# aluo-x/3D_SLN

Measured on AMD Instinct MI355X. Metric: scene-graph VAE steps/sec + 256² diff-render fps, 1/2/4/8 MI355X, higher is better.
Workload: dtype f32; 1 GPU; BASELINE configs[1]: batch=64 scene graphs x (32 objects, 64 triples) per GPU, Sg2ScVAE train step at train.py defaults (embedding_dim=64, 5+5 GraphTripleConv, BatchNorm); O=2048, T=4096, hipgraph=True, distinct_batches_cycled=4, eps=N(0,1) drawn on the device inside the step, parallelism=dp1

## Files before the change

### 3d_sln_amd/_lib.py

```python
from __future__ import annotations

import ctypes as C
import os

HERE = os.path.dirname(os.path.abspath(__file__))
LIB_PATH = os.path.join(HERE, "libsln_hip.so")

SLN_E = {-1: "SLN_E_BADARG", -2: "SLN_E_UNSUPPORTED", -3: "SLN_E_STATE", -4: "SLN_E_NOGPU", -5: "SLN_E_NOMEM", -6: "SLN_E_CAPTURE"}

c_f32p = C.c_void_p
c_i64p = C.c_void_p


class SlnError(RuntimeError):
    pass


class SlnVaeConfig(C.Structure):
    _fields_ = [(n, C.c_int) for n in (
        "embedding_dim", "gconv_num_layers", "recurrent", "batch_norm", "decoder_cat", "use_ae",
        "box_dim", "n_angle", "num_objs", "num_preds", "num_attrs", "no_attr")]


class SlnVaeUnit(C.Structure):
# ... 115 lines not shown
class SlnDbgEmbed(C.Structure):
    _fields_ = [(n, C.c_void_p) for n in ("objs", "attrs", "angles", "boxes", "obj_emb", "attr_emb", "angle_emb", "wb", "bb", "mu", "logvar", "eps",
                                          "z_in", "z", "x0", "dx0", "d_obj_emb", "d_attr_emb", "d_angle_emb", "d_wb", "d_bb", "dz", "idx", "src",
                                          "dst", "src2", "dst2", "st_objs", "st_attrs", "st_angles", "st_boxes", "attrs32", "deg", "err",
                                          "zero_ptr")] + [("zero_bytes", C.c_int64)] + \
               [(n, C.c_int) for n in ("kind", "O", "n_obj", "n_attr", "n_box", "n_angle", "box_dim", "n_z", "use_ae", "z_in_x0", "rows_obj",
                                       "rows_attr", "rows_angle", "ld", "col0", "n", "table_rows", "T", "n2", "pad_")]


class SlnDbgOpt(C.Structure):
    _fields_ = [(n, C.c_void_p) for n in ("params", "grads", "m", "v", "total_loss")] + [("pro", C.POINTER(SlnDbgEmbed))] + \
               [("n", C.c_int64), ("step", C.c_int64), ("seed", C.c_uint64), ("offset", C.c_uint64)] + \
               [(n, C.c_float) for n in ("lr", "beta1", "beta2", "eps")] + [("kind", C.c_int), ("calls", C.c_int)] + \
               [("out_step", C.c_int64), ("out_offset", C.c_uint64), ("out_bc1", C.c_float), ("out_bc2", C.c_float), ("out_skip", C.c_int),
                ("pad_", C.c_int)]


class SlnViewPlace(C.Structure):
    _fields_ = [(n, C.c_void_p) for n in ("bank_v", "bank_f", "voff", "foff", "voff_host", "foff_host", "A", "tr", "row_model", "row_label",
                                          "shell_v", "shell_f", "shell_f_host", "shell_label", "K", "Rm", "t")] + \
               [(n, C.c_int32) for n in ("M", "Vtot", "Ftot", "Fm", "Vs", "Fs", "R", "V", "N", "reserved")] + \
               [("orig_size", C.c_float), ("near", C.c_float)]


class SlnReproject(C.Structure):
    _fields_ = [(n, C.c_void_p) for n in ("depth_src", "k_src", "pose", "K_tgt")] + \
               [(n, C.c_int32) for n in ("B", "Hs", "Ws", "reserved")] + \
               [(n, C.c_float) for n in ("orig_size", "near", "gap", "reserved_f")]


class SlnDraw3D(C.Structure):
    _fields_ = [(n, C.c_void_p) for n in ("faces_xyz", "face_index", "depth", "face_label", "chosen", "K", "light_cam", "albedo")] + \
               [(n, C.c_int32) for n in ("R", "V", "F", "S", "k", "shadows")] + \
               [(n, C.c_float) for n in ("ambient", "intensity", "min_dist", "bias")] + [("background", C.c_float * 3)]


SIGNATURES = {
    "sln_version": (C.c_int, []),
    "sln_build_arch": (C.c_char_p, []),
    "sln_device_ok": (C.c_int, []),
    "sln_vae_num_units": (C.c_int, [C.POINTER(SlnVaeConfig)]),
    "sln_vae_create": (C.c_int, [C.POINTER(SlnVaeConfig), C.POINTER(C.c_void_p)]),
    "sln_vae_destroy": (None, [C.c_void_p]),
    "sln_vae_workspace_bytes": (C.c_int64, [C.c_void_p, C.c_int, C.c_int]),
    "sln_vae_bind": (C.c_int, [C.c_void_p, C.POINTER(SlnVaeTensors), C.c_void_p, C.c_int64, C.c_int, C.c_int]),
    "sln_vae_set_batch": (C.c_int, [C.c_void_p, C.POINTER(SlnVaeBatch), C.c_void_p]),
    "sln_vae_check_batch": (C.c_int, [C.c_void_p, C.c_void_p]),
    "sln_vae_encoder": (C.c_int, [C.c_void_p, c_f32p, c_f32p, C.c_int, C.c_void_p]),
    "sln_vae_decoder": (C.c_int, [C.c_void_p, c_f32p, c_f32p, c_f32p, C.c_int, C.c_void_p]),
    "sln_vae_forward": (C.c_int, [C.c_void_p, c_f32p, c_f32p, c_f32p, c_f32p, c_f32p, c_f32p, C.c_int, C.c_void_p]),
    "sln_vae_loss": (C.c_int, [C.c_void_p, c_f32p, c_f32p, c_f32p, c_f32p, C.c_float, c_f32p, C.c_int, C.c_void_p]),
    "sln_vae_decoder_backward": (C.c_int, [C.c_void_p, c_f32p, c_f32p, c_f32p, C.c_void_p]),
    "sln_vae_encoder_backward": (C.c_int, [C.c_void_p, c_f32p, c_f32p, C.c_void_p]),
    "sln_vae_backward": (C.c_int, [C.c_void_p, C.c_void_p]),
    "sln_vae_params_changed": (C.c_int, [C.c_void_p]),
    "sln_vae_zero_grad": (C.c_int, [C.c_void_p, C.c_void_p]),
    "sln_vae_adam_step": (C.c_int, [C.c_void_p, C.c_float, C.c_void_p]),
    "sln_vae_adam_reset": (C.c_int, [C.c_void_p, C.c_int64, C.c_void_p]),
    "sln_vae_adam_get_step": (C.c_int, [C.c_void_p, C.POINTER(C.c_int64), C.c_void_p]),
    "sln_vae_set_grad_guard": (C.c_int, [C.c_void_p, c_f32p]),
    "sln_vae_seed": (C.c_int, [C.c_void_p, C.c_uint64, C.c_uint64, C.c_void_p]),
    "sln_vae_last_eps": (C.c_int, [C.c_void_p, c_f32p, C.c_void_p]),
    "sln_vae_randn": (C.c_int, [C.c_void_p, c_f32p, C.c_int64, C.c_void_p]),
    "sln_layout_heatmap": (C.c_int, [c_f32p, C.c_int64, C.c_int, C.c_int, C.c_int, C.c_int, c_f32p, C.c_void_p]),
    "sln_vae_set_training": (C.c_int, [C.c_void_p, C.c_int]),
    "sln_vae_set_gemm_precision": (C.c_int, [C.c_void_p, C.c_int]),
    "sln_vae_train_step": (C.c_int, [C.c_void_p, c_f32p, C.c_float, C.c_float, c_f32p, C.c_int, C.c_int, C.c_void_p]),
    "sln_vae_group_create": (C.c_int, [C.POINTER(C.c_void_p), C.c_int, C.POINTER(SlnVaeGroupIO), C.POINTER(C.c_void_p)]),
    "sln_vae_group_decoder": (C.c_int, [C.c_void_p, C.c_void_p]),
    "sln_vae_group_decoder_backward": (C.c_int, [C.c_void_p, C.c_void_p]),
    "sln_vae_group_launches": (C.c_int, [C.c_void_p, C.POINTER(C.c_int), C.POINTER(C.c_int), C.POINTER(C.c_int)]),
    "sln_vae_group_transposes": (C.c_int64, [C.c_void_p]),
    "sln_vae_group_fused_params": (C.c_int, [C.c_void_p, C.POINTER(C.c_void_p), C.POINTER(C.c_int64), C.c_int]),
    "sln_vae_group_destroy": (None, [C.c_void_p]),
    "sln_debug_side_stream": (C.c_int, [C.c_void_p, C.POINTER(C.c_int), C.POINTER(C.c_int)]),
    "sln_side_stream_prepare": (C.c_int, [C.c_void_p]),
    "sln_side_stream_forget": (C.c_int, [C.c_void_p]),
    "sln_prof_enable": (C.c_int, [C.c_int]),
    "sln_set_deterministic": (C.c_int, [C.c_int]),
    "sln_get_deterministic": (C.c_int, []),
    "sln_set_store_policy": (C.c_int, [C.c_int]),
    "sln_get_store_policy": (C.c_int, []),
    "sln_parse_store_policy_env": (C.c_int, [C.c_char_p, C.c_int]),
    "sln_debug_tn_plan": (C.c_int, [C.c_void_p, C.c_void_p, C.c_void_p, C.c_int, C.c_void_p, C.c_void_p, C.c_int]),
    "sln_debug_tn_plan_mixed": (C.c_int, [C.c_void_p, C.c_void_p, C.c_void_p, C.c_void_p, C.c_int, C.c_void_p, C.c_void_p, C.c_int]),
    "sln_prof_read": (C.c_int, [C.c_void_p, C.c_void_p, C.c_void_p, C.c_int]),
    "sln_vae_tap": (C.c_int64, [C.c_void_p, C.c_int, C.c_int, c_f32p, C.c_void_p]),
    "sln_gconv_workspace_bytes": (C.c_int64, [C.c_int, C.c_int, C.c_int, C.c_int, C.c_int, C.c_int]),
    "sln_gconv_forward": (C.c_int, [C.c_int, C.c_int, C.c_int, C.c_int, C.c_int, C.c_int, C.POINTER(SlnVaeUnit), c_f32p, c_f32p,
                                    C.c_void_p, C.c_int, C.c_int, C.c_int, C.c_void_p, C.c_int64, c_f32p, c_f32p, C.c_void_p]),
    "sln_gconv_net_create": (C.c_int, [C.c_int, C.c_int, C.c_int, C.c_int, C.c_int, C.c_int, C.POINTER(C.c_void_p)]),
    "sln_gconv_net_set_edges": (C.c_int, [C.c_void_p, C.c_void_p, C.c_int, C.c_int, C.c_void_p]),
    "sln_gconv_net_forward": (C.c_int, [C.c_void_p, c_f32p, c_f32p, c_f32p, c_f32p, C.c_int, C.c_void_p]),
    "sln_gconv_net_backward": (C.c_int, [C.c_void_p, c_f32p, c_f32p, c_f32p, c_f32p, C.c_void_p]),
    "sln_linear_forward": (C.c_int, [c_f32p, C.c_int, C.c_int, c_f32p, c_f32p, c_f32p, C.c_int, C.c_void_p,
                                     C.c_int, C.c_void_p]),
    "sln_linear_wgrad": (C.c_int, [c_f32p, c_f32p, C.c_int, C.c_int, C.c_int, c_f32p, c_f32p, C.c_void_p]),
    "sln_debug_gemm_nt": (C.c_int, [C.POINTER(SlnDbgGemmNT), C.c_int, C.POINTER(C.c_int), C.c_void_p]),
    "sln_debug_gemm_tn": (C.c_int, [C.POINTER(SlnDbgGemmTN), C.c_int, C.c_int, C.c_void_p]),
    "sln_debug_gemm_tn_mixed": (C.c_int, [C.POINTER(SlnDbgGemmTN), C.c_int, C.c_void_p]),
    "sln_debug_gemm_nt_route": (C.c_int, [C.POINTER(SlnDbgGemmNT), C.POINTER(SlnDbgNTRoute)]),
    "sln_debug_gemm_nt_half": (C.c_int, [C.POINTER(SlnDbgGemmNT), C.c_int, C.c_void_p]),
    "sln_debug_gemm_nt_half_takes": (C.c_int, [C.POINTER(SlnDbgGemmNT)]),
    "sln_debug_gemm_sizes": (C.c_int, [C.POINTER(C.c_int), C.c_int]),
    "sln_debug_vae_csr": (C.c_int, [c_i64p, C.c_int, C.c_int, C.c_int, C.POINTER(SlnDbgCsr), C.c_void_p, C.c_void_p]),
    "sln_debug_vae_edge": (C.c_int, [C.POINTER(SlnDbgEdge), C.c_int, C.c_int, C.POINTER(C.c_int), C.c_void_p]),
    "sln_debug_vae_loss": (C.c_int, [C.POINTER(SlnDbgLoss), C.c_void_p]),
    "sln_debug_vae_tables": (C.c_int, [C.c_int, C.c_void_p, C.c_int, C.c_int, C.c_float, C.c_int, C.c_int, C.c_int, C.c_void_p]),
    "sln_debug_vae_embed": (C.c_int, [C.POINTER(SlnDbgEmbed), C.c_int, C.c_int, C.POINTER(C.c_int), C.c_void_p]),
    "sln_debug_vae_opt": (C.c_int, [C.POINTER(SlnDbgOpt), C.c_void_p]),
    "sln_debug_vae_sizes": (C.c_int, [C.POINTER(C.c_int), C.c_int]),
    "sln_debug_vae_leaf_launches": (C.c_int64, [C.c_void_p]),
    "sln_debug_vae_half_launches": (C.c_int64, [C.c_void_p]),
    "sln_debug_vae_tail_launches": (C.c_int64, [C.c_void_p]),
    "sln_debug_vae_graph_captures": (C.c_int64, [C.c_void_p]),
    "sln_project_faces": (C.c_int, [c_f32p, C.c_void_p, c_f32p, c_f32p, c_f32p, C.c_int, C.c_int, C.c_int, C.c_float, C.c_float, c_f32p, C.c_void_p]),
    "sln_project_faces_backward": (C.c_int, [c_f32p, C.c_void_p, c_f32p, c_f32p, c_f32p, C.c_int, C.c_int, C.c_int, C.c_float, C.c_float, c_f32p,
                                             c_f32p, C.c_void_p]),
    "sln_raster_workspace_bytes": (C.c_int64, [C.c_int, C.c_int]),
    "sln_raster_forward": (C.c_int, [c_f32p, C.c_int, C.c_int, C.c_int, C.c_float, C.c_float, C.c_void_p, C.c_void_p,
                                     c_f32p, c_f32p, C.c_void_p]),
    "sln_raster_forward_dual": (C.c_int, [c_f32p, C.c_int, C.c_int, C.c_int, C.c_float, C.c_float, C.c_float, C.c_void_p,
                                          C.c_void_p, c_f32p, c_f32p, C.c_void_p, c_f32p, c_f32p, C.c_void_p]),
    "sln_raster_texture_sample": (C.c_int, [c_f32p, c_f32p, C.c_void_p, c_f32p, c_f32p, C.c_int, C.c_int, C.c_int, C.c_int,
                                            C.c_float, c_f32p, C.c_void_p]),
    "sln_raster_backward_depth": (C.c_int, [c_f32p, C.c_void_p, c_f32p, c_f32p, c_f32p, C.c_int, C.c_int, C.c_int, c_f32p,
                                            C.c_void_p]),
    "sln_raster_backward_rgb": (C.c_int, [c_f32p, C.c_void_p, c_f32p, c_f32p, C.c_int, C.c_int, C.c_int, C.c_int, C.c_float,
                                          c_f32p, C.c_void_p]),
    "sln_raster_texture_sample_chw": (C.c_int, [c_f32p, c_f32p, C.c_void_p, c_f32p, c_f32p, C.c_int, C.c_int, C.c_int, C.c_int, C.c_int,
                                                C.c_float, C.c_float, c_f32p, C.c_void_p]),
    "sln_raster_backward_rgb_multi": (C.c_int, [c_f32p, C.c_void_p, C.c_void_p, C.c_void_p, C.c_int, C.c_int, C.c_int, C.c_int, C.c_float,
                                                C.c_void_p, c_f32p, C.c_void_p]),
    "sln_scene_workspace_bytes": (C.c_int64, [C.c_int, C.c_int, C.c_int]),
    "sln_scene_forward": (C.c_int, [c_f32p, C.c_void_p, C.c_int, C.c_int, C.c_int, C.c_int, C.c_void_p, C.c_void_p,
                                    C.c_float, C.c_float, C.c_float, C.c_float, C.c_void_p, c_f32p, C.c_void_p]),
    "sln_scene_forward_live": (C.c_int, [c_f32p, C.c_void_p, C.c_int, C.c_int, C.c_int, C.c_int, C.c_void_p, C.c_void_p,
                                         C.c_float, C.c_float, C.c_float, C.c_float, C.c_void_p, c_f32p, C.c_void_p, C.c_void_p, C.c_void_p]),
    "sln_spade_prepare": (C.c_int, [C.c_void_p]),
    "sln_spade_release": (C.c_int, [C.c_void_p, C.c_int]),
    "sln_spade_conv": (C.c_int, [c_f32p, C.c_int, C.c_int, C.c_int, C.c_int, c_f32p, c_f32p, C.c_int, C.c_int, C.c_int, C.c_int,
                                 C.c_float, c_f32p, C.c_void_p]),
    "sln_spade_modulate": (C.c_int, [c_f32p, C.c_int, C.c_int, C.c_int, C.c_int, c_f32p, c_f32p, C.c_int, C.c_int, c_f32p, c_f32p,
                                     C.c_int, C.c_float, c_f32p, C.c_void_p]),
    "sln_layernorm_stats": (C.c_int, [c_f32p, C.c_int, C.c_int64, C.c_float, C.c_void_p, c_f32p, C.c_void_p]),
    "sln_spade_apply": (C.c_int, [c_f32p, c_f32p, C.c_int, C.c_int, C.c_int, C.c_int, C.c_int, c_f32p, C.c_int, C.c_float, c_f32p, C.c_void_p]),
    "sln_spade_apply_up": (C.c_int, [c_f32p, C.c_int, c_f32p, C.c_int, C.c_int, C.c_int, C.c_int, C.c_int, c_f32p, C.c_int, C.c_float, c_f32p,
                                     C.c_void_p]),
    "sln_resize": (C.c_int, [c_f32p, C.c_int, C.c_int, C.c_int, C.c_int, C.c_int, C.c_int, c_f32p, C.c_void_p]),
    "sln_spade_depth_concat": (C.c_int, [c_f32p, C.c_int, C.c_int, C.c_int, C.c_int, c_f32p, c_f32p, C.c_int, c_f32p, C.c_int, C.c_void_p]),
    "sln_se_scale_add": (C.c_int, [c_f32p, c_f32p, C.c_int, C.c_int, C.c_int64, c_f32p, c_f32p, c_f32p, c_f32p, C.c_void_p]),
    "sln_spade_conv_sums": (C.c_int, [c_f32p, C.c_int, C.c_int, C.c_int, C.c_int, c_f32p, c_f32p, C.c_int, C.c_int, C.c_int, C.c_int,
                                      C.c_float, c_f32p, C.c_void_p, C.c_void_p, C.c_void_p]),
    "sln_spade_modulate_up": (C.c_int, [c_f32p, C.c_int, C.c_int, C.c_int, C.c_int, c_f32p, c_f32p, C.c_int, C.c_int, c_f32p, C.c_int,
                                        c_f32p, C.c_int, C.c_float, c_f32p, C.c_void_p]),
    "sln_layernorm_finalize": (C.c_int, [C.c_void_p, C.c_int, C.c_int64, C.c_int, C.c_float, c_f32p, C.c_void_p]),
    "sln_spade_conv_f16": (C.c_int, [c_f32p, C.c_int, C.c_int, C.c_int, C.c_int, C.c_void_p, C.c_void_p, c_f32p, C.c_int, C.c_int, C.c_int,
                                     C.c_int, C.c_float, c_f32p, C.c_void_p]),
    "sln_spade_conv_sums_f16": (C.c_int, [c_f32p, C.c_int, C.c_int, C.c_int, C.c_int, C.c_void_p, C.c_void_p, c_f32p, C.c_int, C.c_int,
                                          C.c_int, C.c_int, C.c_float, c_f32p, C.c_void_p, C.c_void_p, C.c_void_p]),
    "sln_spade_modulate_f16": (C.c_int, [c_f32p, C.c_int, C.c_int, C.c_int, C.c_int, C.c_void_p, C.c_void_p, c_f32p, C.c_int, C.c_int,
                                         c_f32p, c_f32p, C.c_int, C.c_float, c_f32p, C.c_void_p]),
    "sln_spade_modulate_up_f16": (C.c_int, [c_f32p, C.c_int, C.c_int, C.c_int, C.c_int, C.c_void_p, C.c_void_p, c_f32p, C.c_int, C.c_int,
                                            c_f32p, C.c_int, c_f32p, C.c_int, C.c_float, c_f32p, C.c_void_p]),
    "sln_block_tail": (C.c_int, [c_f32p, C.c_int, c_f32p, C.c_int, C.c_int, C.c_int, C.c_int, C.c_void_p, c_f32p, c_f32p, c_f32p,
                                 C.c_int, c_f32p, C.c_void_p, C.c_int, C.c_float, c_f32p, C.c_void_p]),
# ... 122 lines not shown
```

### 3d_sln_amd/csrc/gemm_bodies.h

```cpp
#pragma once
#include "sln_common.h"
#include "sln_gemm.h"
#include "sln_prof.h"

#include <cstdlib>
#include <cstring>
#include <type_traits>
namespace {


#ifndef SLN_TRACE
#define SLN_TRACE(i)
#endif
#ifndef SLN_TRACEH
#define SLN_TRACEH(i)
#endif

#ifndef SLN_NT_SCHED
#define SLN_NT_SCHED 1
#endif
#ifndef SLN_TN_SCHED
#define SLN_TN_SCHED 1
#endif
#ifndef SLN_TN_ABL
// ... 1237 lines not shown
        if (n == 0) pieceG(rt, buf, 0, stage_next);
        if (n == 1) pieceG2(rt, 0, stage_next);
        if (n == 2) pieceG(rt, buf, 1, stage_next);
        if (n == 3) { pieceG2(rt, 1, stage_next); rd(buf, 2, S0{}); }
      });
      mma4(S1{}, [&](int n) __attribute__((always_inline)) {
        if (n == 0) pieceX(rt, buf, 0, stage_next);
        if (n == 1) pieceX(rt, buf, 1, stage_next);
        if (n == 2) pieceI(rt, 0, stage_next);
        if (n == 3) { pieceI(rt, 1, stage_next); rd(buf, 3, S1{}); }
      });
      mma4(S0{}, [&](int) __attribute__((always_inline)) {});
      __syncthreads();
      rd(buf ^ 1, 0, S0{});
      SLN_SB;
      mma4(S1{}, [&](int) __attribute__((always_inline)) {});
    };
#undef SLN_SB
    for (int rt = 0; rt < ntiles; rt += 2) { sbody(rt, S1{}); sbody(rt + 1, S0{}); }
  }
#else
  for (int rt = 0; rt < ntiles; rt += 2) { body(rt, S1{}); body(rt + 1, S0{}); }
#endif

  __syncthreads();
  float* red = As;
  {
    float* dst = red + (wave * 16) * 64 + lane;
    if (wr == 0) {
#pragma unroll
      for (int r = 0; r < 16; ++r) dst[r * 64] = tn_acc_read(acc[1][r]);
    } else {
#pragma unroll
      for (int r = 0; r < 16; ++r) dst[r * 64] = tn_acc_read(acc[0][r]);
    }
  }
  __syncthreads();
  {
    const float* src = red + ((wave ^ 2) * 16) * 64 + lane;
    const float sc = a.sgd_step != nullptr ? -a.sgd_step[0] : 1.f;
    const int k = k0 + 32 * wc + lrow;
    float* dcol = a.dW + min(k, a.Kin - 1);
    const bool kv = k < a.Kin;
    if (wr == 0) {
#pragma unroll
      for (int r = 0; r < 16; ++r) {
        const float v = (tn_acc_read(acc[0][r]) + src[r * 64]) * sc;
        const int n = n0 + 2 * ((r & 3) + 8 * (r >> 2) + 4 * lk);
        if (kv && n < a.Nout) sln_gatomic_add(dcol + (size_t)n * a.lddw, v);
      }
    } else {
#pragma unroll
      for (int r = 0; r < 16; ++r) {
        const float v = (src[r * 64] + tn_acc_read(acc[1][r])) * sc;
        const int n = n0 + 2 * ((r & 3) + 8 * (r >> 2) + 4 * lk) + 1;
        if (kv && n < a.Nout) sln_gatomic_add(dcol + (size_t)n * a.lddw, v);
      }
    }
  }

  if (a.db != nullptr && (bx % tiles_k) == 0) {
#pragma unroll
    for (int off = TPRA; off < 64; off <<= 1) {
      dbacc.x += __shfl_xor(dbacc.x, off, 64); dbacc.y += __shfl_xor(dbacc.y, off, 64);
      dbacc.z += __shfl_xor(dbacc.z, off, 64); dbacc.w += __shfl_xor(dbacc.w, off, 64);
    }
    __syncthreads();
    float4* dbs = reinterpret_cast<float4*>(red);
    if (lane < TPRA) dbs[wave * TPRA + lane] = dbacc;
    __syncthreads();
    if (tid < TPRA) {
      const float4 p0 = dbs[tid], p1 = dbs[TPRA + tid], p2 = dbs[2 * TPRA + tid], p3 = dbs[3 * TPRA + tid];
      const int n = n0 + 4 * tid;
      const float sb = a.sgd_step != nullptr ? -a.sgd_step[0] : 1.f;
      if (n + 0 < a.Nout) sln_gatomic_add(a.db + n + 0, (((p0.x + p1.x) + p2.x) + p3.x) * sb);
      if (n + 1 < a.Nout) sln_gatomic_add(a.db + n + 1, (((p0.y + p1.y) + p2.y) + p3.y) * sb);
      if (n + 2 < a.Nout) sln_gatomic_add(a.db + n + 2, (((p0.z + p1.z) + p2.z) + p3.z) * sb);
      if (n + 3 < a.Nout) sln_gatomic_add(a.db + n + 3, (((p0.w + p1.w) + p2.w) + p3.w) * sb);
    }
  }
}


template <bool G_X2>
__device__ __forceinline__ void gemm_tn_mixed_item(const GemmTNArgs* __restrict__ probs, const TnMultiItem it, char* smem) {
  if (it.prob < 0) return;
  if (it.xg) gemm_tn_body<64, 64, 2, 2, G_X2, true>(probs[it.prob], it.tile, it.chunk, smem);
  else gemm_tn_body<64, 64, 2, 2, G_X2, false>(probs[it.prob], it.tile, it.chunk, smem);
}

inline bool tn_gathers(const GemmTNArgs& a) {
  bool g = false;
  for (int s = 0; s < a.X.nseg; ++s) g |= a.X.seg[s].which != 0;
  return g;
}

inline bool tn_supported(const GemmTNArgs& a) {
  for (int s = 0; s < a.G.nseg; ++s) if (a.G.seg[s].which != 0) return false;
  return true;
}

inline size_t nt_smem_bytes(int K, int BM, int BN, int WM) {
  const int kpad = (K + 31) & ~31;
  return (size_t)sln_crows(kpad + 4) * 16 + (size_t)2 * (BM + BN) * (BK + 4) * 4 + (size_t)BN * 16 + (size_t)WM * BN * 16;
}

inline size_t tn_smem_bytes(int BM, int BN) { return (size_t)(BM + BN) * 16 + (size_t)2 * BK * (BM + TN_PAD + BN + TN_PAD) * 4; }

inline int nt_heuristic_tile(const GemmNTArgs& a) {
  static const int forced = std::getenv("SLN_NT_TILE") ? std::atoi(std::getenv("SLN_NT_TILE")) : -1;
  (void)a;
  return forced >= 0 ? forced : 0;
}

inline bool nt_big_shape(const GemmNTArgs& a) {
  return (long)sln_cdiv(a.M, 128) * sln_cdiv(a.N, 64) >= 384;
}

inline bool nt_unaligned(const GemmNTArgs& a) {
  for (int s = 0; s + 1 < a.A.nseg; ++s) if (a.A.seg[s].len % BK) return true;
  return false;
}

inline int nt_amode(const GemmNTArgs& a) {
  bool x2 = false;
  for (int s = 0; s < a.A.nseg; ++s) x2 |= a.A.seg[s].x2 != nullptr;
  bool ident = !x2;
  for (int s = 0; s < a.A.nseg; ++s) ident = ident && a.A.seg[s].coef == SLN_COEF_IDENT;
  return x2 ? 1 : (ident ? 2 : 0);
}

inline bool tn_prepare(GemmTNArgs& a) {
  bool x2 = false;
  for (int s = 0; s < a.G.nseg; ++s) x2 |= a.G.seg[s].x2 != nullptr;
  if (a.rows_per_block <= 0) {
    static const int target = std::getenv("SLN_TN_TARGET") ? std::atoi(std::getenv("SLN_TN_TARGET")) : 768;
    static const int minrows = std::getenv("SLN_TN_MINROWS") ? std::atoi(std::getenv("SLN_TN_MINROWS")) : 256;
    const int tiles = sln_cdiv(a.Nout, 64) * sln_cdiv(a.Kin, 64);
    int chunks = sln_cdiv(target, tiles);
    int rpb = sln_cdiv(sln_cdiv(a.R, chunks), BK) * BK;
    a.rows_per_block = rpb < minrows ? minrows : rpb;
  }
  return x2;
}

}
```

### 3d_sln_amd/csrc/gemm_f32.hip

```cpp
#include <cstdio>
#include <cstdlib>
#include <algorithm>
#include <vector>
#include "gemm_bodies.h"
#include "vae_multi.h"
namespace {
constexpr bool nt_coef_helpers(int amode, int epi) { return amode != 2 || epi == EPI_MASK; }
template <int BM, int BN, int AMODE, int EPI>
constexpr bool nt_helpers() { return BM == 64 && BN == 64 && nt_coef_helpers(AMODE, EPI); }
template <int BM, int BN, int WM, int WN, int AMODE, int EPI, int MULTI, int ST = 0>
__global__ __launch_bounds__((nt_helpers<BM, BN, AMODE, EPI>() ? 512 : 256)) void gemm_nt_kernel(const GemmNTArgs a) {
  extern __shared__ __attribute__((aligned(16))) char smem[];
  gemm_nt_body<BM, BN, WM, WN, AMODE, EPI, MULTI, nt_helpers<BM, BN, AMODE, EPI>(), ST>(a, blockIdx.x, ((a.M + BM - 1) / BM) * ((a.N + BN - 1) / BN), smem);
}

template <int AMODE, int EPI>
constexpr bool nt_helpers2() { return nt_coef_helpers(AMODE, EPI); }
template <int J, int AMODE, int EPI, int ST = 0>
__global__ __launch_bounds__((nt_helpers2<AMODE, EPI>() ? 512 : 256)) void gemm_nt16_kernel(const GemmNTArgs a) {
  extern __shared__ __attribute__((aligned(16))) char smem[];
  gemm_nt_body16<J, AMODE, EPI, nt_helpers2<AMODE, EPI>(), ST>(a, blockIdx.x, ((a.M + 63) / 64) * ((a.N + 32 * J - 1) / (32 * J)), smem);
}

template <int AMODE, int EPI, int NSEG = 1, int ST = 0>
// ... 51 lines not shown
  else hipLaunchKernelGGL((gemm_nt16_kernel<J, AMODE, EPI>), dim3(grid), dim3(nt_helpers2<AMODE, EPI>() ? 512 : 256), smem, st, a);
  SLN_CHECK_LAUNCH();
  return 0;
}

template <int BM, int BN, int WM, int WN, int AMODE, int EPI>
int launch_nt(const GemmNTArgs& a, const NtRoute& rt, hipStream_t st) {
  const size_t smem = nt_smem_bytes(a.K, BM, BN, WM);
  const int grid = sln_cdiv(a.M, BM) * sln_cdiv(a.N, BN);
  if (grid <= 0) return 0;
  if (smem > 48 * 1024) { int r = sln_gemm_init(); if (r) return r; }
  constexpr int NTHR = nt_helpers<BM, BN, AMODE, EPI>() ? 512 : 256;
  if (rt.threads != NTHR) return -3;
#define SLN_NT_GO(ST_)                                                                                                                   \
  if (rt.multi == 2) {                                                                                                                   \
    if constexpr (BM == 64 && BN == 64) hipLaunchKernelGGL((gemm_nt_kernel<64, 64, WM, WN, AMODE, EPI, 2, ST_>), dim3(grid), dim3(NTHR), smem, st, a); \
    else return -2;                                          \
  }                                                                                                                                      \
  else if (rt.multi == 1) hipLaunchKernelGGL((gemm_nt_kernel<BM, BN, WM, WN, AMODE, EPI, 1, ST_>), dim3(grid), dim3(NTHR), smem, st, a); \
  else hipLaunchKernelGGL((gemm_nt_kernel<BM, BN, WM, WN, AMODE, EPI, 0, ST_>), dim3(grid), dim3(NTHR), smem, st, a);
  if (nt_store_mode() == SLN_ST_WT) { SLN_NT_GO(SLN_ST_WT) } else { SLN_NT_GO(SLN_ST_PLAIN) }
#undef SLN_NT_GO
  SLN_CHECK_LAUNCH();
  return 0;
}

template <int AMODE, int EPI>
int launch_nt_route(const GemmNTArgs& a, const NtRoute& rt, hipStream_t st) {
  switch (rt.body) {
    case NT_BODY_SMALL: return launch_nt_small<AMODE, EPI>(a, rt, st);
    case NT_BODY_SMALL3: return launch_nt_small<AMODE, EPI, 3>(a, rt, st);
    case NT_BODY_16J3: return launch_nt16<3, AMODE, EPI>(a, rt, st);
    case NT_BODY_16J5: return launch_nt16<5, AMODE, EPI>(a, rt, st);
    case NT_BODY_128x64: return launch_nt<128, 64, 2, 2, AMODE, EPI>(a, rt, st);
    case NT_BODY_128: return launch_nt<128, 128, 2, 2, AMODE, EPI>(a, rt, st);
    case NT_BODY_64: return launch_nt<64, 64, 2, 2, AMODE, EPI>(a, rt, st);
    default: return -1;
  }
}

NtRoute nt_route(const GemmNTArgs& a, int epi, int tile) {
  static const bool no_small = std::getenv("SLN_NO_SMALL_NT") != nullptr;
  NtRoute r;
  r.amode = nt_amode(a); r.multi = 0;
  if (tile < 0 && !no_small && nt_wants_small(a)) r.body = NT_BODY_SMALL;
  else if (tile < 0 && !no_small && nt_wants_small3(a)) { r.body = NT_BODY_SMALL3; r.multi = 1; }
  else {
    const int J16 = tile < 0 ? nt16_pick(a) : 0;
    if (J16 == 3) r.body = NT_BODY_16J3;
    else if (J16 == 5) r.body = NT_BODY_16J5;
    else {
      if (tile < 0) tile = nt_heuristic_tile(a);
      const bool unaligned = a.A.nseg > 1 && nt_unaligned(a);
      if (unaligned) tile = 0;
      r.body = tile == 1 ? NT_BODY_128x64 : (tile == 2 ? NT_BODY_128 : NT_BODY_64);
      r.multi = a.A.nseg > 1 ? (unaligned ? 2 : 1) : 0;
    }
  }
  const bool big = r.body == NT_BODY_128x64 || r.body == NT_BODY_128;
  r.threads = !big && nt_coef_helpers(r.amode, epi) ? 512 : 256;
  return r;
}

template <int BM, int BN, int WM, int WN, bool G_X2, bool XG>
__global__ __launch_bounds__(256) void gemm_tn_kernel(const GemmTNArgs a) {
  extern __shared__ __attribute__((aligned(16))) char smem[];
  gemm_tn_body<BM, BN, WM, WN, G_X2, XG>(a, blockIdx.x, blockIdx.y, smem);
}

template <bool G_X2, bool XG>
__global__ __launch_bounds__(256) void gemm_tn_multi_kernel(const GemmTNArgs* __restrict__ probs, const TnMultiMeta* __restrict__ meta) {
  extern __shared__ __attribute__((aligned(16))) char smem[];
  const TnMultiItem it = meta->item[blockIdx.x];
  if (it.prob < 0) return;
  gemm_tn_body<64, 64, 2, 2, G_X2, XG>(probs[it.prob], it.tile, it.chunk, smem);
}

template <bool G_X2>
__global__ __launch_bounds__(256) void gemm_tn_mixed_kernel(const GemmTNArgs* __restrict__ probs, const TnMixedMeta* __restrict__ meta) {
  extern __shared__ __attribute__((aligned(16))) char smem[];
  gemm_tn_mixed_item<G_X2>(probs, meta->item[blockIdx.x], smem);
}

template <int BM, int BN, int WM, int WN, bool G_X2>
int launch_tn(const GemmTNArgs& a, hipStream_t st) {
  const size_t smem = tn_smem_bytes(BM, BN);
  const int gx = sln_cdiv(a.Nout, BM) * sln_cdiv(a.Kin, BN);
  const int gy = sln_cdiv(a.R, a.rows_per_block);
  if (gx <= 0 || gy <= 0) return 0;
  if (!tn_supported(a)) return -1;
  if (tn_gathers(a)) hipLaunchKernelGGL((gemm_tn_kernel<BM, BN, WM, WN, G_X2, true>), dim3(gx, gy), dim3(256), smem, st, a);
  else hipLaunchKernelGGL((gemm_tn_kernel<BM, BN, WM, WN, G_X2, false>), dim3(gx, gy), dim3(256), smem, st, a);
  SLN_CHECK_LAUNCH();
  return 0;
}

}

template <int BM, int BN, int WM, int WN, int ST>
static int init_nt_tile() {
  hipError_t e = hipSuccess;
#define SLN_SET(X2, EPI)                                                                                          \
  if (e == hipSuccess)                                                                                            \
    e = hipFuncSetAttribute(reinterpret_cast<const void*>(&gemm_nt_kernel<BM, BN, WM, WN, X2, EPI, 0, ST>),       \
                            hipFuncAttributeMaxDynamicSharedMemorySize, 160 * 1024);                              \
  if (e == hipSuccess)                                                                                            \
    e = hipFuncSetAttribute(reinterpret_cast<const void*>(&gemm_nt_kernel<BM, BN, WM, WN, X2, EPI, 1, ST>),       \
                            hipFuncAttributeMaxDynamicSharedMemorySize, 160 * 1024);                              \
  if (e == hipSuccess && BM == 64 && BN == 64)                                                                    \
    e = hipFuncSetAttribute(reinterpret_cast<const void*>(&gemm_nt_kernel<64, 64, WM, WN, X2, EPI, 2, ST>),       \
                            hipFuncAttributeMaxDynamicSharedMemorySize, 160 * 1024);
  SLN_SET(0, EPI_PLAIN) SLN_SET(0, EPI_STATS) SLN_SET(0, EPI_MASK)
  SLN_SET(1, EPI_PLAIN) SLN_SET(1, EPI_STATS) SLN_SET(1, EPI_MASK)
  SLN_SET(2, EPI_PLAIN) SLN_SET(2, EPI_STATS) SLN_SET(2, EPI_MASK)
#undef SLN_SET
  return (int)e;
}

int sln_gemm_group_init();
int sln_vae_tail_init();
int sln_gemm_init() {
  static bool done = false;
  if (done) return 0;
  int r = init_nt_tile<64, 64, 2, 2, SLN_ST_PLAIN>();
  if (!r) r = init_nt_tile<64, 64, 2, 2, SLN_ST_WT>();
#define SLN_SET_S(AM, EPI)                                                                                        \
  if (!r) r = (int)hipFuncSetAttribute(reinterpret_cast<const void*>(&gemm_nt_small_kernel<AM, EPI, 1>),         \
                                       hipFuncAttributeMaxDynamicSharedMemorySize, 160 * 1024);                  \
  if (!r) r = (int)hipFuncSetAttribute(reinterpret_cast<const void*>(&gemm_nt_small_kernel<AM, EPI, 3>),         \
                                       hipFuncAttributeMaxDynamicSharedMemorySize, 160 * 1024);                  \
  if (!r) r = (int)hipFuncSetAttribute(reinterpret_cast<const void*>(&gemm_nt_small_kernel<AM, EPI, 1, SLN_ST_WT>), \
                                       hipFuncAttributeMaxDynamicSharedMemorySize, 160 * 1024);                  \
  if (!r) r = (int)hipFuncSetAttribute(reinterpret_cast<const void*>(&gemm_nt_small_kernel<AM, EPI, 3, SLN_ST_WT>), \
                                       hipFuncAttributeMaxDynamicSharedMemorySize, 160 * 1024);
  SLN_SET_S(0, EPI_PLAIN) SLN_SET_S(0, EPI_STATS) SLN_SET_S(0, EPI_MASK) SLN_SET_S(1, EPI_PLAIN) SLN_SET_S(1, EPI_STATS)
  SLN_SET_S(1, EPI_MASK) SLN_SET_S(2, EPI_PLAIN) SLN_SET_S(2, EPI_STATS) SLN_SET_S(2, EPI_MASK)
#undef SLN_SET_S
#define SLN_SET_16(J, AM, EPI)                                                                                    \
  if (!r) r = (int)hipFuncSetAttribute(reinterpret_cast<const void*>(&gemm_nt16_kernel<J, AM, EPI>),             \
                                       hipFuncAttributeMaxDynamicSharedMemorySize, 160 * 1024);                  \
  if (!r) r = (int)hipFuncSetAttribute(reinterpret_cast<const void*>(&gemm_nt16_kernel<J, AM, EPI, SLN_ST_WT>),  \
                                       hipFuncAttributeMaxDynamicSharedMemorySize, 160 * 1024);
#define SLN_SET_16J(J)                                                                                            \
  SLN_SET_16(J, 0, EPI_PLAIN) SLN_SET_16(J, 0, EPI_STATS) SLN_SET_16(J, 0, EPI_MASK) SLN_SET_16(J, 1, EPI_PLAIN) SLN_SET_16(J, 1, EPI_STATS) \
  SLN_SET_16(J, 1, EPI_MASK) SLN_SET_16(J, 2, EPI_PLAIN) SLN_SET_16(J, 2, EPI_STATS) SLN_SET_16(J, 2, EPI_MASK)
  SLN_SET_16J(3) SLN_SET_16J(5)
#undef SLN_SET_16J
#undef SLN_SET_16
  if (!r) r = init_nt_tile<128, 64, 2, 2, SLN_ST_PLAIN>();
  if (!r) r = init_nt_tile<128, 64, 2, 2, SLN_ST_WT>();
  if (!r) r = init_nt_tile<128, 128, 2, 2, SLN_ST_PLAIN>();
  if (!r) r = init_nt_tile<128, 128, 2, 2, SLN_ST_WT>();
#define SLN_SET_TN(X2, XG)                                                                                        \
  if (!r) r = (int)hipFuncSetAttribute(reinterpret_cast<const void*>(&gemm_tn_kernel<64, 64, 2, 2, X2, XG>),     \
                                       hipFuncAttributeMaxDynamicSharedMemorySize, 160 * 1024);
  SLN_SET_TN(true, true) SLN_SET_TN(true, false) SLN_SET_TN(false, true) SLN_SET_TN(false, false)
#undef SLN_SET_TN
#define SLN_SET_TNM(X2, XG)                                                                                       \
  if (!r) r = (int)hipFuncSetAttribute(reinterpret_cast<const void*>(&gemm_tn_multi_kernel<X2, XG>),             \
                                       hipFuncAttributeMaxDynamicSharedMemorySize, 160 * 1024);
  SLN_SET_TNM(true, true) SLN_SET_TNM(true, false) SLN_SET_TNM(false, true) SLN_SET_TNM(false, false)
#undef SLN_SET_TNM
  if (!r) r = (int)hipFuncSetAttribute(reinterpret_cast<const void*>(&gemm_tn_mixed_kernel<true>), hipFuncAttributeMaxDynamicSharedMemorySize, 160 * 1024);
  if (!r) r = (int)hipFuncSetAttribute(reinterpret_cast<const void*>(&gemm_tn_mixed_kernel<false>), hipFuncAttributeMaxDynamicSharedMemorySize, 160 * 1024);
  if (!r) r = sln_gemm_group_init();
  if (!r) r = sln_vae_tail_init();
  done = r == 0;
  return r;
}




int sln_launch_gemm_nt(const GemmNTArgs& a, int epi, int tile, hipStream_t st) {
  SlnProfScope prof(SLN_FAM_GEMM_NT, 2.0 * a.M * a.N * a.K, st);
  const NtRoute rt = nt_route(a, epi, tile);
  static const bool nt_log = std::getenv("SLN_NT_LOG") != nullptr;
  if (nt_log) std::fprintf(stderr, "NTLOG M=%d N=%d K=%d amode=%d epi=%d nseg=%d\n", a.M, a.N, a.K, rt.amode, epi, a.A.nseg);
#define SLN_DISPATCH(AM)                                                              \
  if (rt.amode == AM) {                                                               \
    if (epi == EPI_MASK) return launch_nt_route<AM, EPI_MASK>(a, rt, st);             \
    if (epi == EPI_STATS) return launch_nt_route<AM, EPI_STATS>(a, rt, st);           \
    return launch_nt_route<AM, EPI_PLAIN>(a, rt, st);                                 \
  }
  SLN_DISPATCH(0) SLN_DISPATCH(1) SLN_DISPATCH(2)
#undef SLN_DISPATCH
  return -1;
}

int sln_plan_nt_small(const GemmNTArgs& a, int epi, int* tiles) {
  static const bool no_small = std::getenv("SLN_NO_SMALL_NT") != nullptr;
  if (no_small || a.M <= 0 || a.N <= 0) return -1;
  int nseg = 0;
  const int amode = nt_amode(a);
  if (amode == 1 || epi == EPI_STATS) return -1;
  if (nt_wants_small(a)) nseg = 1;
  else if (nt_wants_small3(a)) nseg = 3;
  if (nseg) { *tiles = sln_cdiv(a.M, 32) * sln_cdiv(a.N, 32); return amode * 16 + epi * 4 + nseg; }
  if (nt_big_shape(a)) return -1;
  *tiles = sln_cdiv(a.M, 64) * sln_cdiv(a.N, 64);
  return 1000 + amode * 16 + epi * 4 + (a.A.nseg > 1 ? (nt_unaligned(a) ? 2 : 1) : 0);
}

template <int AMODE, int EPI, int NSEG>
static int launch_nt_small_multi(const GemmNTArgs* tab, const int* tiles, int R, int max_tiles, size_t smem, hipStream_t st) {
  static bool raised = false;
  if (smem > 48 * 1024 && !raised) {
    hipError_t e = hipFuncSetAttribute(reinterpret_cast<const void*>(&gemm_nt_small_multi_kernel<AMODE, EPI, NSEG>),
                                       hipFuncAttributeMaxDynamicSharedMemorySize, 160 * 1024);
    if (e != hipSuccess) return (int)e;
    raised = true;
  }
  hipLaunchKernelGGL((gemm_nt_small_multi_kernel<AMODE, EPI, NSEG>), dim3(max_tiles, R), dim3(nt_helpers2<AMODE, EPI>() ? 512 : 256), smem, st, tab, tiles);
  SLN_CHECK_LAUNCH();
  return 0;
}

template <int AMODE, int EPI, int MULTI>
static int launch_nt64_multi(const GemmNTArgs* tab, const int* tiles, int R, int max_tiles, size_t smem, hipStream_t st) {
  static bool raised = false;
  if (smem > 48 * 1024 && !raised) {
    hipError_t e = hipFuncSetAttribute(reinterpret_cast<const void*>(&gemm_nt64_multi_kernel<AMODE, EPI, MULTI>),
                                       hipFuncAttributeMaxDynamicSharedMemorySize, 160 * 1024);
    if (e != hipSuccess) return (int)e;
    raised = true;
  }
  hipLaunchKernelGGL((gemm_nt64_multi_kernel<AMODE, EPI, MULTI>), dim3(max_tiles, R), dim3(nt_helpers<64, 64, AMODE, EPI>() ? 512 : 256), smem, st, tab, tiles);
  SLN_CHECK_LAUNCH();
  return 0;
}

int sln_launch_gemm_nt_small_multi(const GemmNTArgs* tab, const int* tiles_dev, int R, int key, int max_tiles, int max_K, double flops,
                                   hipStream_t st) {
  if (R <= 0 || max_tiles <= 0) return 0;
  SlnProfScope prof(SLN_FAM_GEMM_NT, flops, st);
  if (key >= 1000) {
    const size_t smem64 = nt_smem_bytes(max_K, 64, 64, 2);
    const int am = (key - 1000) / 16, ep = ((key - 1000) / 4) % 4, mu = (key - 1000) % 4;
#define SLN_NT64M(AM, EP, MU) if (am == AM && ep == EP && mu == MU) return launch_nt64_multi<AM, EP, MU>(tab, tiles_dev, R, max_tiles, smem64, st);
    SLN_NT64M(0, EPI_PLAIN, 0) SLN_NT64M(0, EPI_PLAIN, 1) SLN_NT64M(0, EPI_PLAIN, 2) SLN_NT64M(0, EPI_MASK, 0) SLN_NT64M(0, EPI_MASK, 1) SLN_NT64M(0, EPI_MASK, 2)
    SLN_NT64M(2, EPI_PLAIN, 0) SLN_NT64M(2, EPI_PLAIN, 1) SLN_NT64M(2, EPI_PLAIN, 2) SLN_NT64M(2, EPI_MASK, 0) SLN_NT64M(2, EPI_MASK, 1) SLN_NT64M(2, EPI_MASK, 2)
#undef SLN_NT64M
    return -1;
  }
  const size_t smem = nt_small_smem_bytes(max_K);
  const int amode = key / 16, epi = (key / 4) % 4, nseg = key % 4;
#define SLN_NTM(AM, EP, NS) if (amode == AM && epi == EP && nseg == NS) return launch_nt_small_multi<AM, EP, NS>(tab, tiles_dev, R, max_tiles, smem, st);
// ... 9 lines not shown
  const bool x2 = tn_prepare(a);
  if (x2) return launch_tn<64, 64, 2, 2, true>(a, st);
  return launch_tn<64, 64, 2, 2, false>(a, st);
}

static int tn_plan(GemmTNArgs* probs, int n, int max_probs, int max_items, bool mixed, int* nprob, int* nblocks, TnMultiItem* item,
                   int* blocks, bool* x2, bool* xg, double* flops) {
  if (n < 1 || n > max_probs) return -1;
  static const int target0 = std::getenv("SLN_TN_MULTI_ROWS") ? std::atoi(std::getenv("SLN_TN_MULTI_ROWS")) : 768;
  static const bool no_xcd = std::getenv("SLN_TN_NO_XCD") != nullptr;
  bool any_x2 = false, any_xg = false;
  double work = 0.0;
  for (int i = 0; i < n; ++i) {
    const GemmTNArgs& a = probs[i];
    if (a.R <= 0 || a.Nout <= 0 || a.Kin <= 0 || !tn_supported(a)) return -1;
    for (int s = 0; s < a.G.nseg; ++s) any_x2 |= a.G.seg[s].x2 != nullptr;
    any_xg |= tn_gathers(a);
    work += 2.0 * a.R * a.Nout * a.Kin;
  }
  struct Group { int prob, chunk, tiles; long cost; };
  std::vector<Group> groups;
  int per_xcd[8];
  std::vector<int> owner;
  for (long target = g_sln_deterministic ? (1L << 30) : (target0 > 0 ? target0 : 1024);; target *= 2) {
    groups.clear();
    for (int i = 0; i < n; ++i) {
      GemmTNArgs& a = probs[i];
      const int chunks = sln_cdiv(a.R, (int)(target > a.R ? a.R : target));
      a.rows_per_block = sln_cdiv(sln_cdiv(a.R, chunks), BK) * BK;
      const int tiles = sln_cdiv(a.Nout, 64) * sln_cdiv(a.Kin, 64), nch = sln_cdiv(a.R, a.rows_per_block);
      for (int c = 0; c < nch; ++c) {
        const int rows = (c + 1) * a.rows_per_block <= a.R ? a.rows_per_block : a.R - c * a.rows_per_block;
        groups.push_back(Group{i, c, tiles, (long)tiles * rows});
      }
    }
    std::stable_sort(groups.begin(), groups.end(), [](const Group& x, const Group& y) { return x.cost > y.cost; });
    long load[8] = {0, 0, 0, 0, 0, 0, 0, 0};
    for (int x = 0; x < 8; ++x) per_xcd[x] = 0;
    owner.assign(groups.size(), 0);
    for (size_t g = 0; g < groups.size(); ++g) {
      int best = 0;
      if (no_xcd) best = (int)(g % 8);
      else for (int x = 1; x < 8; ++x) if (load[x] < load[best]) best = x;
      owner[g] = best; load[best] += groups[g].cost; per_xcd[best] += groups[g].tiles;
    }
    int mx = 0;
    for (int x = 0; x < 8; ++x) mx = per_xcd[x] > mx ? per_xcd[x] : mx;
    if (8 * mx <= max_items) break;
    if (mixed || target > (1L << 30)) return -1;
  }
  if (any_xg && !mixed) {
    const int* any = nullptr;
    for (int i = 0; i < n; ++i) { if (probs[i].X.idx_a) any = probs[i].X.idx_a; else if (probs[i].X.idx_b) any = probs[i].X.idx_b; }
    for (int i = 0; i < n; ++i) if (!probs[i].X.idx_a && !probs[i].X.idx_b) probs[i].X.idx_a = any;
  }
  int mx = 0;
  for (int x = 0; x < 8; ++x) mx = per_xcd[x] > mx ? per_xcd[x] : mx;
  *nprob = n; *nblocks = 8 * mx;
  std::memset(item, 0, sizeof(TnMultiItem) * (size_t)(mixed ? 8 * mx : max_items));
  for (int b = 0; b < 8 * mx; ++b) item[b].prob = -1;
  int fill[8] = {0, 0, 0, 0, 0, 0, 0, 0};
  for (size_t g = 0; g < groups.size(); ++g) {
    const int x = owner[g];
    const int gathers = mixed && tn_gathers(probs[groups[g].prob]) ? 1 : 0;
    for (int t = 0; t < groups[g].tiles; ++t) {
      TnMultiItem& it = item[8 * (fill[x]++) + x];
      it.prob = groups[g].prob; it.tile = t; it.chunk = groups[g].chunk; it.xg = gathers;
    }
  }
  *blocks = 8 * mx; *x2 = any_x2; *xg = any_xg; *flops = work;
  return 0;
}

int sln_tn_multi_plan(GemmTNArgs* probs, int n, TnMultiMeta* meta, int* blocks, bool* x2, bool* xg, double* flops) {
  return tn_plan(probs, n, SLN_TN_MULTI_MAX, SLN_TN_MULTI_ITEMS, false, &meta->nprob, &meta->nblocks, meta->item, blocks, x2, xg, flops);
}

int sln_tn_mixed_plan(GemmTNArgs* probs, int n, TnMixedMeta* meta, int* blocks, bool* x2, double* flops) {
  bool xg = false;
  return tn_plan(probs, n, SLN_TN_MIXED_MAX, SLN_TN_MIXED_ITEMS, true, &meta->nprob, &meta->nblocks, meta->item, blocks, x2, &xg, flops);
}

int sln_launch_gemm_tn_multi(const GemmTNArgs* dev_probs, const TnMultiMeta* dev_meta, int blocks, bool x2, bool xg, double flops,
                             hipStream_t st) {
  if (blocks <= 0) return 0;
  SlnProfScope prof(SLN_FAM_GEMM_TN, flops, st);
  const size_t smem = tn_smem_bytes(64, 64);
  if (smem > 48 * 1024) { int r = sln_gemm_init(); if (r) return r; }
  if (x2 && xg) hipLaunchKernelGGL((gemm_tn_multi_kernel<true, true>), dim3(blocks), dim3(256), smem, st, dev_probs, dev_meta);
  else if (x2) hipLaunchKernelGGL((gemm_tn_multi_kernel<true, false>), dim3(blocks), dim3(256), smem, st, dev_probs, dev_meta);
  else if (xg) hipLaunchKernelGGL((gemm_tn_multi_kernel<false, true>), dim3(blocks), dim3(256), smem, st, dev_probs, dev_meta);
  else hipLaunchKernelGGL((gemm_tn_multi_kernel<false, false>), dim3(blocks), dim3(256), smem, st, dev_probs, dev_meta);
  SLN_CHECK_LAUNCH();
  return 0;
}

int sln_launch_gemm_tn_mixed(const GemmTNArgs* dev_probs, const TnMixedMeta* dev_meta, int blocks, bool x2, double flops, hipStream_t st) {
  if (blocks <= 0) return 0;
  SlnProfScope prof(SLN_FAM_GEMM_TN, flops, st);
  const size_t smem = tn_smem_bytes(64, 64);
  if (smem > 48 * 1024) { int r = sln_gemm_init(); if (r) return r; }
  if (x2) hipLaunchKernelGGL((gemm_tn_mixed_kernel<true>), dim3(blocks), dim3(256), smem, st, dev_probs, dev_meta);
  else hipLaunchKernelGGL((gemm_tn_mixed_kernel<false>), dim3(blocks), dim3(256), smem, st, dev_probs, dev_meta);
  SLN_CHECK_LAUNCH();
  return 0;
}

extern "C" int sln_debug_tn_plan(const int* R, const int* Nout, const int* Kin, int n, int* rows_per_block, int* items, int max_items) {
  if (!R || !Nout || !Kin || !rows_per_block || !items || n < 1 || n > SLN_TN_MULTI_MAX) return -1;
  static thread_local GemmTNArgs probs[SLN_TN_MULTI_MAX];
  static thread_local TnMultiMeta meta;
  std::memset(probs, 0, sizeof(GemmTNArgs) * (size_t)n);
  for (int i = 0; i < n; ++i) {
    probs[i].R = R[i]; probs[i].Nout = Nout[i]; probs[i].Kin = Kin[i];
    probs[i].G.nseg = 1; probs[i].X.nseg = 1; probs[i].lddw = i;
  }
  int blocks = 0; bool x2 = false, xg = false; double flops = 0.0;
  const int r = sln_tn_multi_plan(probs, n, &meta, &blocks, &x2, &xg, &flops);
  if (r) return r;
  if (blocks > max_items) return -2;
  for (int i = 0; i < n; ++i) rows_per_block[probs[i].lddw] = probs[i].rows_per_block;
  for (int b = 0; b < blocks; ++b) {
    const TnMultiItem& it = meta.item[b];
    items[3 * b] = it.prob < 0 ? -1 : probs[it.prob].lddw; items[3 * b + 1] = it.tile; items[3 * b + 2] = it.chunk;
  }
  return blocks;
}

extern "C" int sln_debug_tn_plan_mixed(const int* R, const int* Nout, const int* Kin, const int* gathers, int n, int* rows_per_block,
                                       int* items, int max_items) {
  if (!R || !Nout || !Kin || !gathers || !rows_per_block || !items || n < 1 || n > SLN_TN_MIXED_MAX) return -1;
  std::vector<GemmTNArgs> probs((size_t)n);
  std::vector<TnMixedMeta> meta(1);
  std::memset(probs.data(), 0, sizeof(GemmTNArgs) * (size_t)n);
  for (int i = 0; i < n; ++i) {
    probs[i].R = R[i]; probs[i].Nout = Nout[i]; probs[i].Kin = Kin[i];
    probs[i].G.nseg = 1; probs[i].X.nseg = 1; probs[i].X.seg[0].which = gathers[i] ? 1 : 0; probs[i].lddw = i;
  }
  int blocks = 0; bool x2 = false; double flops = 0.0;
  const int r = sln_tn_mixed_plan(probs.data(), n, meta.data(), &blocks, &x2, &flops);
  if (r) return r;
  if (blocks > max_items) return -2;
  for (int i = 0; i < n; ++i) rows_per_block[probs[i].lddw] = probs[i].rows_per_block;
  for (int b = 0; b < blocks; ++b) {
    const TnMultiItem& it = meta[0].item[b];
    items[4 * b] = it.prob < 0 ? -1 : probs[it.prob].lddw; items[4 * b + 1] = it.tile; items[4 * b + 2] = it.chunk; items[4 * b + 3] = it.xg;
  }
  return blocks;
}

#include "sln_debug.h"

bool sln_dbg_bn(const SlnDbgBn& d, int coef, BnView& v) {
  std::memset(&v, 0, sizeof(v));
  v.sums = d.sums; v.gsums = d.gsums; v.gamma = d.gamma; v.beta = d.beta; v.rmean = d.rmean; v.rvar = d.rvar;
  v.cstride = d.cstride; v.mode = d.mode; v.n_rows = d.n_rows; v.eps = d.eps;
  v.rn = 1.0 / (double)(d.n_rows > 0.f ? d.n_rows : 1.f);
  if (coef == SLN_COEF_IDENT || d.mode == SLN_BN_NONE) return d.mode >= SLN_BN_NONE && d.mode <= SLN_BN_EVAL;
  const bool bwd = coef == SLN_COEF_BWD;
  if (d.mode == SLN_BN_TRAIN) return d.gamma && d.sums && d.cstride > 0 && d.n_rows >= 1.f && (bwd ? d.gsums != nullptr : d.beta != nullptr);
  if (d.mode == SLN_BN_EVAL) return d.gamma && d.rvar && (bwd || (d.beta && d.rmean));
  return false;
}

namespace {

bool dbg_operand(const SlnDbgOperand& d, int rows, int cols, bool gather_ok, bool x2_ok, Operand& op, bool ragged_ok = false) {
  std::memset(&op, 0, sizeof(op));
  if (d.nseg < 1 || d.nseg > 3 || rows <= 0) return false;
  int tot = 0;
  for (int s = 0; s < d.nseg; ++s) {
    const SlnDbgSeg& g = d.seg[s];
    Seg& o = op.seg[s];
    const bool ragged = ragged_ok && s == d.nseg - 1 && (g.len & 3);
    const int len4 = (g.len + 3) & ~3;
    if (!g.x1 || g.len <= 0 || ((g.len & 3) && !ragged)) return false;
    if ((g.ld1 & 3) || (g.c1 & 3) || g.c1 < 0 || g.ld1 < g.c1 + len4) return false;
    if (g.coef < SLN_COEF_IDENT || g.coef > SLN_COEF_BWD || g.which < 0 || g.which > 2) return false;
    if (g.which && (!gather_ok || !(g.which == 1 ? d.idx_a : d.idx_b))) return false;
    if (g.x2) {
      if (!x2_ok || g.coef != SLN_COEF_BWD || (g.ld2 & 3) || (g.c2 & 3) || g.c2 < 0 || g.ld2 < g.c2 + len4) return false;
    } else if (g.coef == SLN_COEF_BWD && g.bn.mode == SLN_BN_TRAIN) return false;
    if (g.coef == SLN_COEF_BWD && !x2_ok) return false;
    o.x1 = g.x1; o.x2 = g.x2; o.ld1 = g.ld1; o.ld2 = g.ld2; o.c1 = g.c1; o.c2 = g.c2; o.len = g.len; o.which = g.which; o.coef = g.coef;
// ... 125 lines not shown
```

### 3d_sln_amd/csrc/prof.hip

```cpp
#include <cstdlib>
#include <vector>
#include "../../include/sln_hip.h"
#include "sln_prof.h"
#include "sln_common.h"

bool g_sln_prof_on = false;
int sln_parse_store_policy(const char* v, int dflt) {
  if (!v || !*v) return dflt;
  char* end = nullptr;
  const long x = std::strtol(v, &end, 10);
  if (*end != 0 || x < 0 || (x & ~(long)SLN_STORE_ALL)) return dflt;
  return (int)x;
}
int g_sln_store_policy = sln_parse_store_policy(std::getenv("SLN_STORE_POLICY"), SLN_STORE_DEFAULT);
int g_sln_deterministic = [] { const char* v = std::getenv("SLN_DETERMINISTIC"); return (v && v[0] == '1') ? 1 : 0; }();

namespace {
struct Rec { int family; double work; hipEvent_t a, b; };
std::vector<Rec> g_recs;
std::vector<hipEvent_t> g_pool;
hipEvent_t take_event() {
  if (!g_pool.empty()) { hipEvent_t e = g_pool.back(); g_pool.pop_back(); return e; }
  hipEvent_t e = nullptr;
  (void)hipEventCreate(&e);
  return e;
}
}

void sln_prof_begin(int family, double work, hipStream_t st) {
  Rec r; r.family = family; r.work = work; r.a = take_event(); r.b = take_event();
  (void)hipEventRecord(r.a, st);
  g_recs.push_back(r);
}
void sln_prof_end(hipStream_t st) {
  if (!g_recs.empty()) (void)hipEventRecord(g_recs.back().b, st);
}

extern "C" int sln_set_deterministic(int on) { g_sln_deterministic = on != 0; return 0; }
extern "C" int sln_get_deterministic(void) { return g_sln_deterministic; }
extern "C" int sln_set_store_policy(int bits) {
  if (bits < 0 || (bits & ~SLN_STORE_ALL)) return SLN_E_BADARG;
  g_sln_store_policy = bits;
  return 0;
}
extern "C" int sln_get_store_policy(void) { return g_sln_store_policy; }
extern "C" int sln_parse_store_policy_env(const char* value, int dflt) { return sln_parse_store_policy(value, dflt); }
extern "C" int sln_prof_enable(int enable) {
  g_sln_prof_on = enable != 0;
  return 0;
}

extern "C" int sln_prof_read(double* ms, double* work, int64_t* launches, int n) {
  if (!ms || !work || !launches || n <= 0) return SLN_E_BADARG;
  for (int i = 0; i < n; ++i) { ms[i] = 0.0; work[i] = 0.0; launches[i] = 0; }
  for (auto& r : g_recs) {
    float t = 0.f;
    hipError_t e = hipEventSynchronize(r.b);
    if (e == hipSuccess) e = hipEventElapsedTime(&t, r.a, r.b);
    if (e == hipSuccess && r.family >= 0 && r.family < n) { ms[r.family] += t; work[r.family] += r.work; launches[r.family] += 1; }
    g_pool.push_back(r.a); g_pool.push_back(r.b);
  }
  g_recs.clear();
  return 0;
}
```

### 3d_sln_amd/csrc/sln_common.h

```cpp
#pragma once
#include <hip/hip_runtime.h>
#include <stdint.h>

#include <cstdlib>

#define SLN_WAVE 64

typedef float f32x16 __attribute__((ext_vector_type(16)));
typedef float f32x4 __attribute__((ext_vector_type(4)));

enum { SLN_BN_NONE = 0, SLN_BN_TRAIN = 1, SLN_BN_EVAL = 2 };

struct BnView {
  const double* sums;
  const double* gsums;
  const float* gamma;
  const float* beta;
  const float* rmean;
  const float* rvar;
  int cstride;
  int mode;
  float n_rows;
  float eps;
  double rn;
// ... 124 lines not shown
  float4 r;
  const float NEG = -3.0e38f;
  if (s.coef == SLN_COEF_IDENT) { r = make_float4(1.f, 0.f, 0.f, NEG); }
  else if (s.coef == SLN_COEF_BWD) {
    float p0, p1, p2; bn_bwd_coef(s.bn, c, p0, p1, p2);
    r = make_float4(p0, p1, p2, NEG);
  } else {
    float sc, sh; bn_fwd_coef(s.bn, c, sc, sh);
    r = make_float4(sc, 0.f, sh, s.coef == SLN_COEF_FWD ? 0.f : NEG);
  }
  return r;
}

__device__ __forceinline__ bool sln_seg_fwd_train(const Seg& s) { return (s.coef == SLN_COEF_FWD || s.coef == SLN_COEF_FWD_NORELU) && s.bn.mode == SLN_BN_TRAIN; }
__device__ __forceinline__ float4 sln_fwd_train_coef(const Seg& g, float gamma, float beta, double s1, double s2) {
  float mean, istd;
  bn_train_mean_istd(g.bn, s1, s2, mean, istd);
  const float scale = gamma * istd;
  return make_float4(scale, 0.f, beta - mean * scale, g.coef == SLN_COEF_FWD ? 0.f : -3.0e38f);
}
__host__ __device__ __forceinline__ int sln_cidx(int c) { return c + (c >> 4); }
__host__ __device__ __forceinline__ int sln_crows(int cols) { return cols + ((cols + 15) >> 4); }

template <int NSEG_MAX = 0>
__device__ __forceinline__ void sln_fill_coefs(const Operand& op, float4* coef, int tid, int nthreads) {
  if (NSEG_MAX == 1) {
    const Seg& g = op.seg[0];
    for (int c = tid; c < g.len; c += nthreads) coef[sln_cidx(c)] = sln_coef_for(g, c);
    return;
  }
  if (NSEG_MAX == 3 && op.nseg == 3 && sln_seg_fwd_train(op.seg[0]) && sln_seg_fwd_train(op.seg[1]) && sln_seg_fwd_train(op.seg[2]) &&
      op.seg[0].len > 0 && op.seg[1].len > 0 && op.seg[2].len > 0) {
    float ga[3], be[3]; double s1[3], s2[3];
#pragma unroll
    for (int s = 0; s < 3; ++s) {
      const BnView& b = op.seg[s].bn;
      const int c = min(tid, op.seg[s].len - 1);
      ga[s] = sln_ldf(b.gamma + c); be[s] = sln_ldf(b.beta + c); s1[s] = sln_ldd(b.sums + c); s2[s] = sln_ldd(b.sums + b.cstride + c);
    }
    int base = 0;
#pragma unroll
    for (int s = 0; s < 3; ++s) {
      const int len = op.seg[s].len;
      const float4 v = sln_fwd_train_coef(op.seg[s], ga[s], be[s], s1[s], s2[s]);
      if (tid < len) coef[sln_cidx(base + tid)] = v;
      for (int c = tid + nthreads; c < len; c += nthreads) coef[sln_cidx(base + c)] = sln_coef_for(op.seg[s], c);
      base += len;
    }
    return;
  }
  int base = 0;
#pragma unroll
  for (int s = 0; s < 3; ++s) {
    if (s < op.nseg) {
      for (int c = tid; c < op.seg[s].len; c += nthreads) coef[sln_cidx(base + c)] = sln_coef_for(op.seg[s], c);
      base += op.seg[s].len;
    }
  }
}

#define SLN_Q_FWD 1048576.0
#define SLN_Q_BWD 17592186044416.0
#define SLN_Q_LOSS 16777216.0
__device__ __forceinline__ double sln_qd(double v, double scale) { return rint(v * scale) * (1.0 / scale); }
__device__ __forceinline__ double sln_q_fwd(int M) {
  const int lg = M > 1 ? 32 - __builtin_clz((unsigned)(M - 1)) : 0;
  const int k = 33 - lg > 20 ? 33 - lg : 20;
  return (double)(1ull << k);
}

__device__ __forceinline__ float wave_sum_halves(float v) {
  return v + __shfl_xor(v, 32, 64);
}

enum { SLN_STORE_PLAIN = 0, SLN_STORE_NT_WT = 1, SLN_STORE_ALL = 1, SLN_STORE_DEFAULT = SLN_STORE_NT_WT };
extern int g_sln_store_policy;
enum { SLN_ST_PLAIN = 0, SLN_ST_WT = 1 };
template <int ST>
__device__ __forceinline__ void sln_st_y(float* p, float v) {
  if (ST == SLN_ST_WT) __hip_atomic_store((float __attribute__((address_space(1)))*)p, v, __ATOMIC_RELAXED, __HIP_MEMORY_SCOPE_AGENT);
  else *p = v;
}

static inline int sln_cdiv(int a, int b) { return (a + b - 1) / b; }

template <typename T>
__global__ void sln_zero_kernel(T* p, size_t n) {
  const size_t i = (size_t)blockIdx.x * blockDim.x + threadIdx.x;
  if (i < n) p[i] = T{};
}
static inline int sln_zero_async(void* p, size_t bytes, hipStream_t st) {
  if (bytes < 4) return 0;
  if (reinterpret_cast<uintptr_t>(p) % 16 == 0 && bytes % 16 == 0) {
    const size_t n = bytes / 16;
    hipLaunchKernelGGL(sln_zero_kernel<uint4>, dim3((unsigned)((n + 255) / 256)), dim3(256), 0, st, static_cast<uint4*>(p), n);
  } else {
    const size_t n = bytes / 4;
    hipLaunchKernelGGL(sln_zero_kernel<uint32_t>, dim3((unsigned)((n + 255) / 256)), dim3(256), 0, st, static_cast<uint32_t*>(p), n);
  }
  return (int)hipGetLastError();
}

#define SLN_CHECK_LAUNCH()                                                  \
  do {                                                                      \
    hipError_t e__ = hipGetLastError();                                     \
    if (e__ != hipSuccess) return (int)e__;                                 \
  } while (0)

hipStream_t sln_overlapping_stream(hipStream_t main);
inline bool sln_capturing(hipStream_t st) {
  hipStreamCaptureStatus cs = hipStreamCaptureStatusNone;
  return hipStreamIsCapturing(st, &cs) == hipSuccess && cs != hipStreamCaptureStatusNone;
}
```

### 3d_sln_amd/csrc/sln_gemm.h

```cpp
#pragma once
#include "sln_common.h"

enum { EPI_PLAIN = 0, EPI_STATS = 1, EPI_MASK = 2 };

struct GemmNTArgs {
  Operand A;
  const float* W;
  const float* bias;
  float* Y;
  int ldy, ycol0;
  int M, N, K, ldw;
  const float* addend;
  int ldadd, addcol0;
  double* osums;
  int ocstride;
  int ldx, xcol0;
  const float* xprev;
  double* ogsums;
  BnView obn;
};

struct GemmTNArgs {
  Operand G;
  Operand X;
  float* dW;
  float* db;
  int lddw;
  int R, Nout, Kin;
  int rows_per_block;
  const float* sgd_step;
};

int sln_launch_gemm_nt(const GemmNTArgs& a, int epi, int tile, hipStream_t st);
int sln_launch_gemm_tn(const GemmTNArgs& a, hipStream_t st);
bool sln_nt_half_takes(const GemmNTArgs& a, int epi);
int sln_launch_gemm_nt_half(const GemmNTArgs& a, int terms, hipStream_t st);
int sln_launch_gemm_group(const GemmNTArgs* nt, const int* epi, int n_nt, hipStream_t st);
enum { SLN_TN_MULTI_MAX = 64, SLN_TN_MULTI_ITEMS = 4096 };
struct TnMultiItem { int prob, tile, chunk, xg; };
struct TnMultiMeta { int nprob, nblocks; TnMultiItem item[SLN_TN_MULTI_ITEMS]; };
enum { SLN_TN_MIXED_MAX = 128, SLN_TN_MIXED_ITEMS = 16384 };
struct TnMixedMeta { int nprob, nblocks; TnMultiItem item[SLN_TN_MIXED_ITEMS]; };
int sln_tn_multi_plan(GemmTNArgs* probs, int n, TnMultiMeta* meta, int* blocks, bool* x2, bool* xg, double* flops);
int sln_launch_gemm_tn_multi(const GemmTNArgs* dev_probs, const TnMultiMeta* dev_meta, int blocks, bool x2, bool xg, double flops,
                             hipStream_t st);
int sln_tn_mixed_plan(GemmTNArgs* probs, int n, TnMixedMeta* meta, int* blocks, bool* x2, double* flops);
int sln_launch_gemm_tn_mixed(const GemmTNArgs* dev_probs, const TnMixedMeta* dev_meta, int blocks, bool x2, double flops, hipStream_t st);
int sln_gemm_init();
```

### 3d_sln_amd/csrc/vae_engine.hip

```cpp
#include <cstddef>
#include <new>
#include <type_traits>
#include <utility>
#include <vector>
#include <cstring>
#include <cstdlib>

#include "../../include/sln_hip.h"
#include "sln_gemm.h"
#include "vae_kernels.h"
#include "vae_multi.h"
#include "sln_prof.h"

namespace {

enum { SK_DEC_ASSEMBLE = 0, SK_EMBED_GATHER, SK_NT, SK_SCATTER_FWD, SK_TN, SK_TN_FLUSH, SK_MASK_GSTATS, SK_ADD2, SK_EMBED_BWD,
       SK_SCATTER_BWD, SK_GATHER_BWD, SK_DEC_ASSEMBLE_BWD, SK_COPY2D };
struct RecStep {
  int kind = -1, epi = 0, idx64 = 0;
  GemmNTArgs nt; GemmTNArgs tn;
  MScatterFwd sf; MScatterBwd sb; MGatherBwd gb; MMaskGstats mg; MDecAssemble da; DecAssembleBwd dab; MEmbedGather eg; MEmbedBwd eb; MAdd2 a2;
};
struct Recorder { std::vector<RecStep> steps; };

// ... 17 lines not shown
  double* sums = nullptr;
  double* gsums = nullptr;
};

struct Layer {
  float *A1 = nullptr, *A2 = nullptr, *M = nullptr, *A3 = nullptr, *A4 = nullptr;
  float *g1 = nullptr, *g2 = nullptr, *g3 = nullptr, *g4 = nullptr;
  int bn[4] = {-1, -1, -1, -1};
  int u0 = 0;
  int D = 0;
  int Do = 0;
  bool first = false, last = false;
  int net = 0;
};

struct Bump {
  char* base; size_t off = 0; bool dry;
  explicit Bump(void* b) : base(static_cast<char*>(b)), dry(b == nullptr) {}
  template <typename T> T* take(size_t n) {
    off = (off + 255) & ~size_t(255);
    T* p = dry ? nullptr : reinterpret_cast<T*>(base + off);
    off += n * sizeof(T);
    return p;
  }
};

}

struct SlnVae {
  SlnVaeConfig cfg;
  int E, H, L, nmod, n_obj_e, n_attr_e, n_box_e, n_angle_e, Dec, Ddc;
  std::vector<Unit> units;
  SlnVaeTensors t;
  bool bound = false;
  int maxO = 0, maxT = 0, O = 0, T = 0;
  SlnVaeBatch batch;
  bool batch_set = false;

  std::vector<Layer> layers;
  std::vector<BnInst> bns;
  int bn_head[6] = {-1, -1, -1, -1, -1, -1};
  int n_bn_enc = 0;

  GraphCsr g;
  int* attrs32 = nullptr; int* err_flag = nullptr;
  double* stats_base = nullptr; size_t stats_doubles = 0, enc_stats_doubles = 0;
  double* gstats_base = nullptr;
  char* zero_begin = nullptr; size_t zero_bytes = 0; bool bulk_zeroed = false;
  bool step_training = true;
  int64_t* st_objs = nullptr; int64_t* st_angles = nullptr; int64_t* st_attrs = nullptr; float* st_boxes = nullptr;
  BnTableEntry* bn_table_dev = nullptr;
  TransposeEntry* tr_table_dev = nullptr; int n_tr = 0, tr_max_tiles = 0;
  AdamScalars* scalars = nullptr; double* loss_acc = nullptr; float* losses = nullptr;
  float *X0e = nullptr, *P0e = nullptr, *X0d = nullptr, *P0d = nullptr;
  float *hbA1 = nullptr, *hbA2 = nullptr, *haA1 = nullptr, *haA2 = nullptr;
  float *mu = nullptr, *logvar = nullptr, *z = nullptr, *eps_buf = nullptr;
  float *bnA1 = nullptr, *anA1 = nullptr, *boxes_pred = nullptr, *logits = nullptr, *angles_pred = nullptr;
  float *dbp = nullptr, *dlogits = nullptr, *g_bn = nullptr, *g_an = nullptr, *d_bx = nullptr, *d_ax = nullptr;
  float *dM = nullptr, *dG[3] = {nullptr, nullptr, nullptr};
  float* dX0_dc = nullptr;
  float *dX0 = nullptr, *dz = nullptr, *dmu = nullptr, *dlv = nullptr;
  float *g_h2 = nullptr, *g_h1 = nullptr, *d_xb = nullptr, *d_xa = nullptr, *tmp_d = nullptr;
  float *g_h2b = nullptr, *g_h1b = nullptr, *tmp_db = nullptr;
  int dbp_ld = 8;

  bool enc_training = false, dec_training = false, have_enc = false, have_dec = false, have_loss_grads = false;
  const float* z_src = nullptr;
  bool z_from_latent = false;
  bool wt_fresh = false;
  float host_kl = 0.f, host_lr = 0.f; int64_t host_step = 0; bool host_scalars_valid = false;
  float* grad_guard = nullptr;
  bool draw_eps = false;
  unsigned long long host_seed[2] = {0, 0};

  struct TnGroup {
    GemmTNArgs probs[SLN_TN_MULTI_MAX]; TnMultiMeta meta; int n = 0, blocks = 0; bool x2 = false, xg = false; double flops = 0.0;
    bool dirty = true; GemmTNArgs* dev_probs = nullptr; TnMultiMeta* dev_meta = nullptr;
  };
  int tn_slots = 32;
  std::vector<GemmTNArgs> tn_kind_scratch;
  bool capturing = false, tn_upload_pending = false;
  int det_seen = 0;
  int store_seen = 0;
  long graph_captures = 0;
  bool tn_per_layer = false;
  int tn_slot_next[3] = {0, 0, 0};
  std::vector<GemmTNArgs> deferred;
  TnGroup* tn_groups_store = nullptr;
  TnGroup& tn_group(int set, int slot, int k) { return tn_groups_store[((size_t)set * tn_slots + slot) * 2 + k]; }
  int upload_group(TnGroup& g) {
    hipError_t e = hipMemcpy(g.dev_probs, g.probs, sizeof(GemmTNArgs) * (size_t)g.n, hipMemcpyHostToDevice);
    if (e == hipSuccess) e = hipMemcpy(g.dev_meta, &g.meta, sizeof(TnMultiMeta), hipMemcpyHostToDevice);
    g.dirty = e != hipSuccess;
    return (int)e;
  }
  bool bn_table_live = false;
  struct TnStage { char* host = nullptr; hipEvent_t done = nullptr; };
  enum { TN_STAGE_SLOTS = 16 };
  TnStage tn_stage[TN_STAGE_SLOTS];
  int tn_stage_next = 0;
  int stage_upload(void* dev0, const void* src0, size_t n0, void* dev1, const void* src1, size_t n1, hipStream_t st) {
    hipStreamCaptureStatus cs = hipStreamCaptureStatusNone;
    if (hipStreamIsCapturing(st, &cs) != hipSuccess || cs != hipStreamCaptureStatusNone) return SLN_E_CAPTURE;
    const size_t cap0 = sizeof(GemmTNArgs) * (size_t)(tn_mixed_store ? SLN_TN_MIXED_MAX : SLN_TN_MULTI_MAX);
    const size_t cap = cap0 + (tn_mixed_store ? sizeof(TnMixedMeta) : sizeof(TnMultiMeta));
    if (n0 > cap0 || n1 > cap - cap0) return SLN_E_BADARG;
    TnStage& sl = tn_stage[tn_stage_next];
    tn_stage_next = (tn_stage_next + 1) % TN_STAGE_SLOTS;
    hipError_t e = hipSuccess;
    if (!sl.host) {
      void* hp = nullptr;
      if (hipHostMalloc(&hp, cap, hipHostMallocDefault) != hipSuccess) return SLN_E_NOMEM;
      sl.host = static_cast<char*>(hp);
      if (hipEventCreateWithFlags(&sl.done, hipEventDisableTiming) != hipSuccess) { (void)hipHostFree(hp); sl.host = nullptr; return SLN_E_NOMEM; }
    } else {
      e = hipEventSynchronize(sl.done);
    }
    if (e == hipSuccess && n0) { std::memcpy(sl.host, src0, n0); e = hipMemcpyAsync(dev0, sl.host, n0, hipMemcpyHostToDevice, st); }
    if (e == hipSuccess && n1) { std::memcpy(sl.host + cap0, src1, n1); e = hipMemcpyAsync(dev1, sl.host + cap0, n1, hipMemcpyHostToDevice, st); }
    if (e == hipSuccess) e = hipEventRecord(sl.done, st);
    return (int)e;
  }
  int upload_group_async(TnGroup& g, hipStream_t st) {
    const int r = stage_upload(g.dev_probs, g.probs, sizeof(GemmTNArgs) * (size_t)g.n, g.dev_meta, &g.meta,
                               offsetof(TnMultiMeta, item) + sizeof(TnMultiItem) * (size_t)g.meta.nblocks, st);
    if (r == 0) g.dirty = false;
    return r;
  }
  int upload_pending_tables() {
    for (int w = 0; w < tn_slots; ++w)
      for (int k = 0; k < 2; ++k) {
        TnGroup& g = tn_group(0, w, k);
        if (g.n > 0 && g.dirty) { int r = upload_group(g); if (r) return r; }
      }
    if (tn_mixed_store && tn_mixed_store[0].n > 0 && tn_mixed_store[0].dirty) { int r = upload_mixed(tn_mixed_store[0]); if (r) return r; }
    tn_upload_pending = false;
    return 0;
  }
  struct TnMixedGroup {
    GemmTNArgs probs[SLN_TN_MIXED_MAX]; TnMixedMeta meta; int n = 0, blocks = 0; bool x2 = false; double flops = 0.0;
    bool dirty = true; GemmTNArgs* dev_probs = nullptr; TnMixedMeta* dev_meta = nullptr;
  };
  TnMixedGroup* tn_mixed_store = nullptr;
  bool tail_merge = true;
  bool it_tail = false;
  bool tail_dec = true;
  bool it_dec_leaf = false;
  bool tail_leaf = true;
  long tail_launches = 0;
  static size_t mixed_meta_bytes(const TnMixedMeta& m) { return offsetof(TnMixedMeta, item) + sizeof(TnMultiItem) * (size_t)m.nblocks; }
  int upload_mixed(TnMixedGroup& g) {
    hipError_t e = hipMemcpy(g.dev_probs, g.probs, sizeof(GemmTNArgs) * (size_t)g.n, hipMemcpyHostToDevice);
    if (e == hipSuccess) e = hipMemcpy(g.dev_meta, &g.meta, mixed_meta_bytes(g.meta), hipMemcpyHostToDevice);
    g.dirty = e != hipSuccess;
    return (int)e;
  }
  enum { TN_MIXED_NO_FIT = 1 << 20 };
  int flush_mixed(int set, const VaeLeaf* leaf, hipStream_t st) {
    if (!tn_mixed_store || !tn_mixed_store[set].dev_probs) return TN_MIXED_NO_FIT;
    TnMixedGroup& tmp = tn_mixed_store[2];
    int n = 0;
    for (const GemmTNArgs& t : deferred) {
      if (t.R <= 0) continue;
      if (n == SLN_TN_MIXED_MAX) return TN_MIXED_NO_FIT;
      tmp.probs[n++] = t;
    }
// ... 1121 lines not shown
                         h->grad_guard ? h->grad_guard : h->losses + 3, st));
  h->wt_fresh = false;
  return 0;
}

int sln_vae_adam_reset(SlnVae* h, int64_t step, void* stream) {
  if (!h || !h->bound) return SLN_E_STATE;
  h->host_step = step;
  return (int)hipMemcpyAsync(&h->scalars->step, &h->host_step, sizeof(int64_t), hipMemcpyHostToDevice, (hipStream_t)stream);
}

int sln_vae_adam_get_step(SlnVae* h, int64_t* step_out, void* stream) {
  if (!h || !h->bound || !step_out) return SLN_E_STATE;
  HIP_RET(hipMemcpyAsync(step_out, &h->scalars->step, sizeof(int64_t), hipMemcpyDeviceToHost, (hipStream_t)stream));
  HIP_RET(hipStreamSynchronize((hipStream_t)stream));
  return 0;
}

int sln_vae_set_grad_guard(SlnVae* h, float* slot) {
  if (!h) return SLN_E_BADARG;
  if (h->grad_guard != slot) { h->grad_guard = slot; h->drop_graphs(); }
  return 0;
}

int sln_vae_seed(SlnVae* h, uint64_t seed, uint64_t offset, void* stream) {
  if (!h || !h->bound) return SLN_E_STATE;
  h->host_seed[0] = seed; h->host_seed[1] = offset;
  HIP_RET(hipMemcpyAsync(&h->scalars->rng_seed, h->host_seed, 2 * sizeof(unsigned long long), hipMemcpyHostToDevice, (hipStream_t)stream));
  return 0;
}

int sln_vae_randn(SlnVae* h, float* out, int64_t n, void* stream) {
  if (!h || !h->bound || !out || n < 0) return SLN_E_BADARG;
  if (n == 0) return 0;
  return sln_launch_randn(out, (long)n, h->scalars, (hipStream_t)stream);
}

int sln_layout_heatmap(const float* boxes_pred, int64_t n_trials, int O, int box_dim, int container_size, int clip_coor, float* counts,
                       void* stream) {
  if (!boxes_pred || !counts || n_trials < 0 || O < 2 || container_size < 2) return SLN_E_BADARG;
  if (box_dim != 6) return SLN_E_UNSUPPORTED;
  return sln_launch_layout_heatmap(boxes_pred, (long)n_trials, O, container_size, clip_coor, counts, (hipStream_t)stream);
}

int sln_vae_last_eps(SlnVae* h, float* eps_out, void* stream) {
  if (!h || !h->batch_set || !eps_out) return SLN_E_STATE;
  return copy_out(eps_out, h->eps_buf, (size_t)h->O * h->E, (hipStream_t)stream);
}

int sln_vae_set_training(SlnVae* h, int training) {
  if (!h) return SLN_E_BADARG;
  if (h->step_training != (training != 0)) { h->step_training = training != 0; h->drop_graphs(); }
  return 0;
}

int sln_vae_set_gemm_precision(SlnVae* h, int mode) {
  if (!h || (mode != 0 && mode != 1 && mode != 3)) return SLN_E_BADARG;
  h->gemm_precision = mode;
  return 0;
}

int sln_vae_params_changed(SlnVae* h) {
  if (!h) return SLN_E_BADARG;
  h->wt_fresh = false;
  return 0;
}

int sln_vae_train_step(SlnVae* h, const float* eps, float kl_weight, float lr, float* losses_out, int use_graph,
                       int with_adam, void* stream) {
  if (!h || !h->batch_set || !h->t.adam_m || !h->t.adam_v) return SLN_E_STATE;
  const int mode = with_adam;
  if (mode < 0 || mode > 3) return SLN_E_BADARG;
  hipStream_t st = (hipStream_t)stream;
  if (mode == SlnVae::TRAIN_ENCODER_BWD) {
    if (!(h->have_dec && h->dec_training == h->step_training && h->z_from_latent)) return SLN_E_STATE;
  } else {
    RET_IF(set_kl(h, kl_weight, lr, st));
    if (eps) RET_IF(copy_out(h->eps_buf, eps, (size_t)h->O * h->E, st));
    const bool draw = !eps && !h->cfg.use_ae;
    if (draw != h->draw_eps) { HIP_RET(hipStreamSynchronize(st)); h->draw_eps = draw; h->drop_graphs(); }
  }
  if (h->det_seen != g_sln_deterministic) { h->det_seen = g_sln_deterministic; h->drop_graphs(); }
  if (h->store_seen != g_sln_store_policy) { h->store_seen = g_sln_store_policy; h->drop_graphs(); }
  if (use_graph && st != nullptr) {
    hipGraphExec_t& ge = h->graph_exec[mode];
    if (!ge || h->graph_O[mode] != h->O || h->graph_T[mode] != h->T) {
      if (ge) { (void)hipGraphExecDestroy(ge); ge = nullptr; }
      HIP_RET(hipStreamSynchronize(st));
      if (mode != SlnVae::TRAIN_ENCODER_BWD) h->wt_fresh = false;
      hipGraph_t graph = nullptr;
      HIP_RET(hipStreamBeginCapture(st, hipStreamCaptureModeThreadLocal));
      h->capturing = true;
      const int r = h->train_iteration(h->eps_buf, mode, st);
      h->capturing = false;
      hipError_t e = hipStreamEndCapture(st, &graph);
      if (r != 0) { if (graph) (void)hipGraphDestroy(graph); return r; }
      if (e != hipSuccess) return (int)e;
      if (h->tn_upload_pending) RET_IF(h->upload_pending_tables());
      e = hipGraphInstantiate(&ge, graph, nullptr, nullptr, 0);
      (void)hipGraphDestroy(graph);
      if (e != hipSuccess) { ge = nullptr; return (int)e; }
      h->graph_O[mode] = h->O; h->graph_T[mode] = h->T;
      ++h->graph_captures;
    }
    HIP_RET(hipGraphLaunch(ge, st));
    h->enc_training = h->dec_training = h->step_training; h->have_enc = h->have_dec = true; h->z_from_latent = true;
    h->wt_fresh = mode == SlnVae::TRAIN_UPTO_DECODER || mode == SlnVae::TRAIN_ENCODER_BWD;
  } else {
    RET_IF(h->train_iteration(h->eps_buf, mode, st));
  }
  if (mode == SlnVae::TRAIN_ENCODER_BWD) return 0;
  RET_IF(copy_out(losses_out, h->losses, 4, st));
  return 0;
}

int sln_gconv_net_create(int D, int H, int Dout, int num_layers, int recurrent, int batch_norm, SlnVae** out) {
  if (!out || D <= 0 || H <= 0 || Dout <= 0 || num_layers < 1 || D % 4 || H % 4 || Dout % 4) return SLN_E_UNSUPPORTED;
  if (Dout != D && num_layers != 1) return SLN_E_UNSUPPORTED;
  SlnVae* h = new (std::nothrow) SlnVae();
  if (!h) return SLN_E_BADARG;
  std::memset(&h->cfg, 0, sizeof(h->cfg));
  h->cfg.gconv_num_layers = num_layers; h->cfg.recurrent = recurrent; h->cfg.batch_norm = batch_norm; h->cfg.decoder_cat = 1;
  h->cfg.box_dim = 4; h->cfg.n_angle = 4; h->cfg.num_preds = 1 << 30;
  h->gconv_only = true;
  h->E = 0; h->H = H; h->L = num_layers; h->nmod = recurrent ? 1 : num_layers;
  h->n_obj_e = h->n_attr_e = h->n_box_e = h->n_angle_e = 0;
  h->Dec = D; h->Ddc = D;
  h->units.resize((size_t)h->nmod * 4);
  for (int m = 0; m < h->nmod; ++m) {
    Unit* u = &h->units[(size_t)m * 4];
    u[0].out = H; u[0].in = 3 * D; u[1].out = 2 * H + Dout; u[1].in = H; u[2].out = H; u[2].in = H; u[3].out = Dout; u[3].in = H;
    for (int k = 0; k < 4; ++k) u[k].bn = batch_norm != 0;
  }
  h->layers.resize(num_layers);
  for (int l = 0; l < num_layers; ++l) {
    Layer& ly = h->layers[l];
    ly.net = 0; ly.first = l == 0; ly.last = l == num_layers - 1; ly.D = D; ly.Do = Dout; ly.u0 = h->unit_of(0, l, 0);
    const int Cs[4] = {H, 2 * H + Dout, H, Dout};
    for (int k = 0; k < 4; ++k) {
      if (!h->units[ly.u0 + k].bn) continue;
      BnInst b; b.unit = ly.u0 + k; b.C = Cs[k]; b.rows = b.rows_code = k < 2 ? -1 : -2;
      ly.bn[k] = (int)h->bns.size(); h->bns.push_back(b);
    }
  }
  h->n_bn_enc = (int)h->bns.size();
  if (read_engine_options(h) != 0) { delete h; return SLN_E_BADARG; }
  h->use_group = false;
  *out = h;
  return 0;
}

int sln_gconv_net_set_edges(SlnVae* h, const int64_t* edges, int O, int T, void* stream) {
  if (!h || !h->bound || !h->gconv_only) return SLN_E_STATE;
  if (O <= 0 || T < 0 || O > h->maxO || T > h->maxT || (T > 0 && !edges)) return SLN_E_BADARG;
  hipStream_t st = (hipStream_t)stream;
  const bool shape_changed = O != h->O || T != h->T || !h->batch_set;
  h->O = O; h->T = T; h->g.T = T; h->g.O = O;
  if (shape_changed) {
    for (auto& ly : h->layers)
      for (int k = 0; k < 4; ++k)
        if (ly.bn[k] >= 0) h->bns[ly.bn[k]].rows = k < 2 ? T : O;
    if (!h->bn_table_live) {
      HIP_RET(hipStreamSynchronize(st));
      RET_IF(upload_bn_table(h));
      h->bn_table_live = true;
    }
// ... 128 lines not shown
    for (std::vector<Launch>* prog : {&fwd, &bwd})
      for (Launch& l : *prog) { fix(l.tab); fix(l.tiles); fix(l.tn_probs); fix(l.tn_meta); }
    stage.clear(); stage.shrink_to_fit();
    return 0;
  }
  ~SlnVaeGroup() {
    for (void* p : allocs) (void)hipFree(p);
    if (ev_fork) (void)hipEventDestroy(ev_fork);
    if (ev_tr) (void)hipEventDestroy(ev_tr);
    if (ev_join) (void)hipEventDestroy(ev_join);
  }
  int fork_side(hipStream_t st) {
    hipError_t e = hipEventRecord(ev_fork, st);
    if (e == hipSuccess) e = hipStreamWaitEvent(side, ev_fork, 0);
    return (int)e;
  }

  int add_single(std::vector<Launch>& prog, const RecStep& st, int room) {
    Launch l; l.kind = L_SINGLE_STEP; l.single = (int)singles.size();
    singles.push_back(st); single_room.push_back(room);
    prog.push_back(l);
    return 0;
  }
  int flush_tn(std::vector<Launch>& prog, std::vector<GemmTNArgs>& pend) {
    static thread_local SlnVae::TnGroup tmp;
    if (!pend.empty()) { Launch f; f.kind = L_FORK; prog.push_back(f); }
    for (int k = 0; k < 2; ++k) {
      std::vector<GemmTNArgs> kind;
      for (const GemmTNArgs& t : pend) if ((int)tn_gathers_host(t) == k) kind.push_back(t);
      size_t next = 0;
      while (next < kind.size()) {
        int want = 0; long tiles = 0;
        for (size_t i = next; i < kind.size() && want < SLN_TN_MULTI_MAX; ++i) {
          const long tl = (long)sln_cdiv(kind[i].Nout, 64) * sln_cdiv(kind[i].Kin, 64);
          if (want > 0 && tiles + tl > SLN_TN_MULTI_ITEMS / 2) break;
          tiles += tl; ++want;
        }
        int r = -1;
        for (; want >= 1; want /= 2) {
          tmp.n = want;
          for (int i = 0; i < want; ++i) tmp.probs[i] = kind[next + i];
          r = sln_tn_multi_plan(tmp.probs, tmp.n, &tmp.meta, &tmp.blocks, &tmp.x2, &tmp.xg, &tmp.flops);
          if (r == 0) break;
        }
        if (r != 0) {
          RecStep st; st.kind = SK_TN; st.tn = kind[next++];
          if (g_sln_deterministic) st.tn.rows_per_block = sln_cdiv(st.tn.R, 32) * 32;
          Launch l; l.kind = L_TN_SINGLE; l.single = (int)singles.size(); l.on_side = true;
          singles.push_back(st); single_room.push_back(-1);
          prog.push_back(l);
          continue;
        }
        next += (size_t)tmp.n;
        Launch l; l.kind = L_TN_MULTI; l.blocks = tmp.blocks; l.x2 = tmp.x2; l.xg = tmp.xg; l.flops = tmp.flops; l.on_side = true;
        std::vector<GemmTNArgs> pv(tmp.probs, tmp.probs + tmp.n);
        RET_IF(upload(pv, &l.tn_probs));
        std::vector<TnMultiMeta> mv(1, tmp.meta);
        RET_IF(upload(mv, &l.tn_meta));
        prog.push_back(l);
      }
    }
    pend.clear();
    return 0;
  }
  static bool tn_gathers_host(const GemmTNArgs& t) {
    bool g = false;
    for (int s2 = 0; s2 < t.X.nseg; ++s2) g |= t.X.seg[s2].which != 0;
    return g;
  }

  int merge(std::vector<Launch>& prog, const std::vector<Recorder>& recs) {
    const size_t n = recs[0].steps.size();
    for (int r = 1; r < R; ++r) {
      if (recs[r].steps.size() != n) return SLN_E_UNSUPPORTED;
      for (size_t s = 0; s < n; ++s) if (recs[r].steps[s].kind != recs[0].steps[s].kind) return SLN_E_UNSUPPORTED;
    }
    std::vector<GemmTNArgs> pend;
    int n_flush = 0;
    for (size_t s = 0; s < n; ++s) {
      const int kind = recs[0].steps[s].kind;
      if (kind == SK_TN) {
        for (int r = 0; r < R; ++r) {
          GemmTNArgs t = recs[r].steps[s].tn;
          if (io.sgd_step != nullptr && t.lddw == t.Kin) {
            for (const Unit& u : eng[r]->units)
              if (u.p.d_weight == t.dW && (t.db == nullptr || u.p.d_bias == t.db)) {
                t.dW = u.p.weight; if (t.db != nullptr) t.db = u.p.bias;
                t.sgd_step = io.sgd_step;
                if (r == 0) {
                  bool listed = false;
                  for (const auto& f : fused) listed = listed || f.first == (const float*)u.p.weight;
                  if (!listed) {
                    fused.push_back(std::make_pair((const float*)u.p.weight, (int64_t)u.out * u.in));
                    if (t.db != nullptr) fused.push_back(std::make_pair((const float*)u.p.bias, (int64_t)u.out));
                  }
                }
                break;
              }
          }
          pend.push_back(t);
        }
        continue;
      }
      if (kind == SK_TN_FLUSH) {
        static const int every = std::getenv("SLN_GROUP_FLUSH_EVERY") ? std::max(1, std::atoi(std::getenv("SLN_GROUP_FLUSH_EVERY"))) : 1;
        bool last = true;
        for (size_t s2 = s + 1; s2 < n; ++s2) if (recs[0].steps[s2].kind == SK_TN) { last = false; break; }
        if (last || ++n_flush % every == 0) RET_IF(flush_tn(prog, pend));
        continue;
      }
      std::vector<int> var(R, -1), gxs(R, 0), gys(R, 0), smf(R, 0);
      std::vector<RecStep> blk(R);
      std::vector<char> asm_blob((size_t)R * SLN_ASM_BLOB);
      for (int r = 0; r < R; ++r) {
        blk[r] = recs[r].steps[s];
        RecStep& b = blk[r];
        switch (kind) {
          case SK_NT: { int t = 0; var[r] = sln_plan_nt_small(b.nt, b.epi, &t); if (var[r] >= 0) var[r] = var[r] * 4 + b.epi * 0; gxs[r] = t; break; }
          case SK_SCATTER_FWD: var[r] = sln_plan_scatter_avg_fwd(b.sf); gxs[r] = b.sf.gx; gys[r] = b.sf.gy; break;
          case SK_SCATTER_BWD: var[r] = sln_plan_scatter_avg_bwd(b.sb); gxs[r] = b.sb.gx; gys[r] = b.sb.gy; break;
          case SK_GATHER_BWD: var[r] = sln_plan_gather_bwd(b.gb); gxs[r] = b.gb.gx; gys[r] = b.gb.gy; break;
          case SK_MASK_GSTATS: var[r] = sln_plan_mask_gstats(b.mg); gxs[r] = b.mg.gx; gys[r] = b.mg.gy; break;
          case SK_DEC_ASSEMBLE: var[r] = sln_plan_dec_assemble(b.da); gxs[r] = b.da.gx; gys[r] = 1; break;
          case SK_EMBED_GATHER: var[r] = sln_plan_embed_gather(b.eg); gxs[r] = b.eg.gx; gys[r] = 1; break;
          case SK_EMBED_BWD: var[r] = sln_plan_embed_bwd(b.eb, b.idx64); gxs[r] = b.eb.gx; gys[r] = b.eb.gy; smf[r] = b.eb.table_rows * b.eb.n; break;
          case SK_ADD2: case SK_COPY2D: var[r] = sln_plan_add2(b.a2); gxs[r] = b.a2.gx; gys[r] = 1; break;
          case SK_DEC_ASSEMBLE_BWD: var[r] = sln_plan_dec_assemble_bwd(b.dab, asm_blob.data() + (size_t)r * SLN_ASM_BLOB, &gxs[r], &smf[r]); gys[r] = 1; break;
          default: return SLN_E_UNSUPPORTED;
        }
      }
      std::vector<bool> done(R, false);
      for (int r0 = 0; r0 < R; ++r0) {
        if (done[r0]) continue;
        if (var[r0] < 0) { done[r0] = true; RET_IF(add_single(prog, recs[r0].steps[s], r0)); continue; }
        std::vector<int> rooms;
        for (int r = r0; r < R; ++r) if (!done[r] && var[r] == var[r0]) { rooms.push_back(r); done[r] = true; }
        Launch l; l.kind = kind; l.variant = var[r0]; l.count = (int)rooms.size();
        for (int r : rooms) { l.gx = gxs[r] > l.gx ? gxs[r] : l.gx; l.gy = gys[r] > l.gy ? gys[r] : l.gy; l.smem_floats = smf[r] > l.smem_floats ? smf[r] : l.smem_floats; }
#define SLN_UP(FIELD, TYPE) { std::vector<TYPE> v; for (int r : rooms) v.push_back(blk[r].FIELD); const TYPE* d = nullptr; RET_IF(upload(v, &d)); l.tab = d; }
        switch (kind) {
          case SK_NT: {
            l.kind = L_NT; l.variant = var[r0] / 4;
            std::vector<GemmNTArgs> v; std::vector<int> tl;
            for (int r : rooms) { v.push_back(blk[r].nt); tl.push_back(gxs[r]); l.maxK = blk[r].nt.K > l.maxK ? blk[r].nt.K : l.maxK; l.flops += 2.0 * blk[r].nt.M * blk[r].nt.N * blk[r].nt.K; }
            const GemmNTArgs* d = nullptr; RET_IF(upload(v, &d)); l.tab = d;
            RET_IF(upload(tl, &l.tiles));
            break;
          }
          case SK_SCATTER_FWD: SLN_UP(sf, MScatterFwd) break;
          case SK_SCATTER_BWD: SLN_UP(sb, MScatterBwd) break;
          case SK_GATHER_BWD: SLN_UP(gb, MGatherBwd) break;
          case SK_MASK_GSTATS: SLN_UP(mg, MMaskGstats) break;
          case SK_DEC_ASSEMBLE: SLN_UP(da, MDecAssemble) break;
          case SK_EMBED_GATHER: SLN_UP(eg, MEmbedGather) break;
          case SK_EMBED_BWD: SLN_UP(eb, MEmbedBwd) break;
          case SK_ADD2: case SK_COPY2D: SLN_UP(a2, MAdd2) break;
          case SK_DEC_ASSEMBLE_BWD: {
            std::vector<char> v;
            for (int r : rooms) v.insert(v.end(), asm_blob.begin() + (size_t)r * SLN_ASM_BLOB, asm_blob.begin() + (size_t)(r + 1) * SLN_ASM_BLOB);
            const char* d = nullptr; RET_IF(upload(v, &d)); l.tab = d;
            break;
          }
        }
#undef SLN_UP
        prog.push_back(l);
      }
    }
    if (!pend.empty()) RET_IF(flush_tn(prog, pend));
    return 0;
  }

  int run(const std::vector<Launch>& prog, hipStream_t st) {
    const bool want_side = use_side;
    static const bool capture_side = std::getenv("SLN_CAPTURE_SIDE") != nullptr;
    side = (want_side && (capture_side || !sln_capturing(st))) ? sln_overlapping_stream(st) : nullptr;
    struct Restore { bool& flag; bool v; ~Restore() { flag = v; } } restore{use_side, want_side};
    if (side == nullptr) use_side = false;
    unsigned long long cap_id = 0;
    {
      hipStreamCaptureStatus cs = hipStreamCaptureStatusNone;
      if (hipStreamGetCaptureInfo(st, &cs, &cap_id) != hipSuccess) { (void)hipGetLastError(); cs = hipStreamCaptureStatusNone; }
      if (cs != hipStreamCaptureStatusActive) cap_id = 0;
    }
    const bool capturing = cap_id != 0;
    if (capturing && &prog == &bwd) bwd_captured = true;
    for (const Launch& l : prog) {
      int r = 0;
      hipStream_t main_st = st;
      hipStream_t st = (l.on_side && use_side) ? side : main_st;
      switch (l.kind) {
        case L_FORK: if (use_side) r = fork_side(main_st); break;
        case L_JOIN:
          if (use_side) { hipError_t e = hipEventRecord(ev_join, side); if (e == hipSuccess) e = hipStreamWaitEvent(main_st, ev_join, 0); r = (int)e; }
          break;
        case L_JOIN_TR:
          if (tr_pending) { r = (int)hipStreamWaitEvent(main_st, ev_tr, 0); tr_pending = false; }
          break;
        case L_NT: r = sln_launch_gemm_nt_small_multi(static_cast<const GemmNTArgs*>(l.tab), l.tiles, l.count, l.variant, l.gx, l.maxK, l.flops, st); break;
        case L_TN_MULTI: r = sln_launch_gemm_tn_multi(l.tn_probs, l.tn_meta, l.blocks, l.x2, l.xg, l.flops, st); break;
        case L_TN_SINGLE: r = sln_launch_gemm_tn(singles[l.single].tn, st); break;
        case L_SINGLE_STEP: r = run_single(singles[l.single], st); break;
        case SK_SCATTER_FWD: r = sln_launch_scatter_avg_fwd_multi(static_cast<const MScatterFwd*>(l.tab), l.count, l.variant, l.gx, l.gy, st); break;
        case SK_SCATTER_BWD: r = sln_launch_scatter_avg_bwd_multi(static_cast<const MScatterBwd*>(l.tab), l.count, l.variant, l.gx, l.gy, st); break;
        case SK_GATHER_BWD: r = sln_launch_gather_bwd_multi(static_cast<const MGatherBwd*>(l.tab), l.count, l.variant, l.gx, l.gy, st); break;
        case SK_MASK_GSTATS: r = sln_launch_mask_gstats_multi(static_cast<const MMaskGstats*>(l.tab), l.count, l.gx, l.gy, st); break;
        case SK_DEC_ASSEMBLE: r = sln_launch_dec_assemble_multi(static_cast<const MDecAssemble*>(l.tab), l.count, l.gx, st); break;
        case SK_EMBED_GATHER: r = sln_launch_embed_gather_multi(static_cast<const MEmbedGather*>(l.tab), l.count, l.gx, st); break;
        case SK_EMBED_BWD: r = sln_launch_embed_bwd_multi(static_cast<const MEmbedBwd*>(l.tab), l.count, l.variant, l.gx, l.gy, l.smem_floats, st); break;
        case SK_ADD2: r = sln_launch_add2_multi(static_cast<const MAdd2*>(l.tab), l.count, l.gx, st); break;
        case SK_COPY2D: r = sln_launch_copy2d_multi(static_cast<const MAdd2*>(l.tab), l.count, l.gx, st); break;
        case SK_DEC_ASSEMBLE_BWD: r = sln_launch_dec_assemble_bwd_multi(l.tab, l.count, l.variant, l.gx, l.smem_floats, st); break;
        case L_ZERO: r = sln_launch_zero_multi(static_cast<const MZero*>(l.tab), l.count, l.max_n16, st); break;
        case L_TRANSPOSE:
          if (l.variant == 1 && (capturing ? wt_capture == cap_id : wt_valid && !bwd_captured)) break;
          r = sln_launch_transpose_table(static_cast<const TransposeEntry*>(l.tab), l.count, l.gx, st);
          if (!r && l.on_side && use_side) { r = (int)hipEventRecord(ev_tr, side); tr_pending = true; }
          if (!r) {
            ++n_transposes;
            if (capturing) wt_capture = l.variant == 0 ? cap_id : 0;
            else wt_valid = true;
          }
          break;
        case L_BN_GRADS: r = sln_launch_bn_param_grads(static_cast<const BnTableEntry*>(l.tab), l.count, l.gx, eng[0]->cfg.recurrent ? 0 : 1, st); break;
        case L_LOG_SOFTMAX: r = sln_launch_log_softmax(logits, io.angles_pred, rows_total, n_angle, st); break;
        case L_LOG_SOFTMAX_BWD: r = sln_launch_log_softmax_bwd(io.angles_pred, io.d_angles_pred, dlogits, rows_total, n_angle, st); break;
        default: r = SLN_E_UNSUPPORTED;
      }
      if (r) return r;
    }
    if (&prog == &bwd) { wt_valid = false; wt_capture = 0; }
    return 0;
  }
  int run_single(const RecStep& b, hipStream_t st) {
    switch (b.kind) {
      case SK_NT: return sln_launch_gemm_nt(b.nt, b.epi, -1, st);
      case SK_SCATTER_FWD: return sln_launch_scatter_avg_fwd(b.sf.A2, b.sf.ld, b.sf.H, b.sf.D, b.sf.bn, b.sf.g, b.sf.O, b.sf.pooled, st);
      case SK_SCATTER_BWD: return sln_launch_scatter_avg_bwd(b.sb.dM, b.sb.dP, b.sb.lddp, b.sb.dpcol0, b.sb.A2, b.sb.ld, b.sb.H, b.sb.D, b.sb.bn, b.sb.g, b.sb.T,
                                                             b.sb.g2, b.sb.gsums, b.sb.cstride, st);
      case SK_GATHER_BWD: return sln_launch_gather_bwd(b.gb.dG, b.gb.ldg, b.gb.D, b.gb.g, b.gb.O, b.gb.add1, b.gb.ldadd1, b.gb.xprev, b.gb.ldx, b.gb.bn,
                                                       b.gb.masked, b.gb.out, b.gb.ldo, b.gb.gsums, b.gb.cstride, st);
      case SK_MASK_GSTATS: return sln_launch_mask_gstats(b.mg.d1, b.mg.ld1, b.mg.d2, b.mg.ld2, b.mg.xprev, b.mg.ldx, b.mg.bn, b.mg.rows, b.mg.cols, b.mg.out,
                                                         b.mg.ldo, b.mg.gsums, b.mg.cstride, st);
      case SK_DEC_ASSEMBLE: return sln_launch_dec_assemble(b.da.a, st);
      case SK_EMBED_GATHER: return sln_launch_embed_gather_i32(b.eg.idx, b.eg.emb, b.eg.rows, b.eg.n, b.eg.out, st);
      case SK_EMBED_BWD: return b.idx64 ? sln_launch_embed_bwd_i64(static_cast<const int64_t*>(b.eb.idx), b.eb.d, b.eb.ld, b.eb.col0, b.eb.rows, b.eb.n, b.eb.table_rows, b.eb.d_emb, st)
                                        : sln_launch_embed_bwd_i32(static_cast<const int*>(b.eb.idx), b.eb.d, b.eb.ld, b.eb.col0, b.eb.rows, b.eb.n, b.eb.table_rows, b.eb.d_emb, st);
      case SK_ADD2: return sln_launch_add2(b.a2.a, b.a2.lda, b.a2.b, b.a2.ldb, b.a2.rows, b.a2.cols, b.a2.out, b.a2.ldo, st);
      case SK_COPY2D: return (int)hipMemcpy2DAsync(b.a2.out, sizeof(float) * b.a2.ldo, b.a2.a, sizeof(float) * b.a2.lda, sizeof(float) * b.a2.cols, (size_t)b.a2.rows,
                                                   hipMemcpyDeviceToDevice, st);
      case SK_DEC_ASSEMBLE_BWD: return sln_launch_dec_assemble_bwd(b.dab, st);
      default: return SLN_E_UNSUPPORTED;
    }
  }
};

extern "C" {

int sln_vae_group_create(SlnVae* const* engines, int R, const SlnVaeGroupIO* io, SlnVaeGroup** out) {
  if (!engines || R < 1 || !io || !out || !io->row0_host || !io->z || !io->boxes_pred || !io->angles_pred || !io->d_boxes_pred ||
      !io->d_angles_pred || !io->dz || io->rows_total < 1) return SLN_E_BADARG;
  for (int r = 0; r < R; ++r) {
    SlnVae* h = engines[r];
    if (!h || !h->bound || !h->batch_set || h->gconv_only) return SLN_E_STATE;
    if (std::memcmp(&h->cfg, &engines[0]->cfg, sizeof(SlnVaeConfig)) != 0) return SLN_E_BADARG;
    if (io->row0_host[r] < 0 || io->row0_host[r] + h->O > io->rows_total) return SLN_E_BADARG;
  }
  SlnVaeGroup* g = new (std::nothrow) SlnVaeGroup();
  if (!g) return SLN_E_NOMEM;
  g->R = R; g->io = *io; g->io.row0_host = nullptr; g->rows_total = io->rows_total; g->n_angle = engines[0]->cfg.n_angle;
  g->eng.assign(engines, engines + R);
  int rc = sln_gemm_init();
  auto fail = [&](int code) { for (SlnVae* h : g->eng) h->rec = nullptr; g->restore_engines(); delete g; return code; };
  if (rc) return fail(rc);
  {
    void* p = nullptr;
    if (hipMalloc(&p, sizeof(float) * (size_t)g->rows_total * g->n_angle * 2) != hipSuccess) return fail(SLN_E_NOMEM);
    g->allocs.push_back(p);
    g->logits = static_cast<float*>(p); g->dlogits = g->logits + (size_t)g->rows_total * g->n_angle;
  }
  std::vector<Recorder> rf(R), rb(R);
  std::vector<MZero> zeros; std::vector<TransposeEntry> trs; std::vector<BnTableEntry> bnt;
  long max_n16 = 0; int tr_tiles = 0, bn_maxc = 0;
// ... 163 lines not shown
```

### 3d_sln_amd/csrc/vae_kernels.hip

```cpp
#include <cstring>
#include "vae_kernels.h"
#include "sln_prof.h"
#include "gemm_bodies.h"

namespace {

constexpr int CB = 64;
constexpr int RL = 4;
constexpr int BOX_ROWS = 64;
constexpr int RB = 32;

__device__ __forceinline__ void commit_col_stats(float s1, float s2, bool valid, double* out, int cstride, int col) {
  __shared__ float red[2][RL][CB];
  red[0][threadIdx.y][threadIdx.x] = s1;
  red[1][threadIdx.y][threadIdx.x] = s2;
  __syncthreads();
  if (threadIdx.y == 0 && valid && out != nullptr) {
    float a = 0.f, b = 0.f;
#pragma unroll
    for (int i = 0; i < RL; ++i) { a += red[0][i][threadIdx.x]; b += red[1][i][threadIdx.x]; }
    atomicAdd(out + col, sln_qd((double)a, SLN_Q_BWD));
    atomicAdd(out + cstride + col, sln_qd((double)b, SLN_Q_BWD));
  }
}
// ... 1250 lines not shown
  hipLaunchKernelGGL(transpose_table_kernel, dim3(max_tiles, n), dim3(256), 0, st, table);
  SLN_CHECK_LAUNCH();
  return 0;
}

int sln_launch_adam(float* params, const float* grads, float* m, float* v, long n, AdamScalars* scalars, const float* total_loss,
                    hipStream_t st) {
  SlnProfScope prof(SLN_FAM_OTHER, 28.0 * n, st);
  long blocks = (n + 4095) / 4096;
  if (blocks > 256) blocks = 256;
  if (blocks < 1) blocks = 1;
  const int vec = ((reinterpret_cast<uintptr_t>(params) | reinterpret_cast<uintptr_t>(grads) | reinterpret_cast<uintptr_t>(m) | reinterpret_cast<uintptr_t>(v)) & 15) == 0;
  hipLaunchKernelGGL(adam_kernel, dim3((unsigned)blocks), dim3(1024), 0, st, params, grads, m, v, n, vec, scalars, total_loss);
  SLN_CHECK_LAUNCH();
  return 0;
}

int sln_launch_randn(float* eps, long n, AdamScalars* scalars, hipStream_t st) {
  if (n <= 0) return 0;
  const long q = (n + 3) / 4;
  hipLaunchKernelGGL(randn_kernel, dim3((unsigned)((q + 255) / 256)), dim3(256), 0, st, eps, n, scalars);
  SLN_CHECK_LAUNCH();
  return 0;
}

int sln_launch_step_prologue(const StepPrologue& a, hipStream_t st) {
  auto blocks = [](long n) { return (unsigned int)((n + 255) / 256); };
  const unsigned int nr = a.eps ? blocks((a.n_eps + 3) / 4) : 0;
  const unsigned int ne = blocks((long)a.enc.O * (a.enc.n_obj + a.enc.n_attr + a.enc.n_box + a.enc.n_angle));
  const unsigned int n1 = blocks((long)a.T * a.n_ec), n2 = blocks((long)a.T * a.n_dc);
  const unsigned int nz = a.zero_ptr ? blocks(a.zero_bytes / 16) : 0;
  const unsigned int nt = (a.tr_tab && a.n_tr > 0 && a.tr_max_tiles > 0) ? (unsigned int)a.n_tr * (unsigned int)a.tr_max_tiles : 0;
  const unsigned int tot = nr + ne + n1 + n2 + nz + nt;
  if (tot == 0) return 0;
  hipLaunchKernelGGL(step_prologue_kernel, dim3(tot), dim3(256), 0, st, a, nr, nr + ne, nr + ne + n1, nr + ne + n1 + n2, nr + ne + n1 + n2 + nz);
  SLN_CHECK_LAUNCH();
  return 0;
}

struct LeafEmbedJob { const void* idx; const float* d; float* d_emb; int ld, col0, rows, n, table_rows, rpb; };
struct LeafArgs {
  AssembleBwdLds asmb, asmb_dc;
  EncAssembleBwd box; int box_gx;
  LeafEmbedJob pdc, pec, attr;
  const BnTableEntry* bn_tab; int bn_n, bn_per_entry, bn_gx, rows_t, rows_o; float mom;
};
__device__ __forceinline__ void vae_leaf_dispatch(const unsigned int b, unsigned int b0, unsigned int b1, unsigned int b2, unsigned int b3,
                                                  unsigned int b4, unsigned int b5, unsigned int b6, const LeafArgs& a) {
  extern __shared__ float tab[];
  if (b < b0) assemble_bwd_lds_body(a.asmb, (int)b);
  else if (b < b1) {
    const int q = (int)(b - b0);
    box_embed_bwd_body(a.box, (int)BOX_ROWS, q % a.box_gx, q / a.box_gx, (int)(threadIdx.x % CB), (int)(threadIdx.x / CB),
                       reinterpret_cast<float (*)[RL][CB]>(tab));
  } else if (b < b2)
    embed_bwd_lds_body<int>(static_cast<const int*>(a.pdc.idx), a.pdc.d, a.pdc.ld, a.pdc.col0, a.pdc.rows, a.pdc.n, a.pdc.table_rows, a.pdc.rpb,
                            a.pdc.d_emb, (int)(b - b1));
  else if (b < b3)
    embed_bwd_lds_body<int>(static_cast<const int*>(a.pec.idx), a.pec.d, a.pec.ld, a.pec.col0, a.pec.rows, a.pec.n, a.pec.table_rows, a.pec.rpb,
                            a.pec.d_emb, (int)(b - b2));
  else if (b < b4)
    embed_bwd_lds_body<int64_t>(static_cast<const int64_t*>(a.attr.idx), a.attr.d, a.attr.ld, a.attr.col0, a.attr.rows, a.attr.n,
                                a.attr.table_rows, a.attr.rpb, a.attr.d_emb, (int)(b - b3));
  else if (b < b5) {
    const int q = (int)(b - b4);
    bn_param_grads_body(a.bn_tab, a.bn_n, a.bn_per_entry, (q % a.bn_gx) * 256 + (int)threadIdx.x, q / a.bn_gx);
  } else if (b < b6) {
    const int q = (int)(b - b5);
    bn_running_update_body(a.bn_tab, a.bn_n, a.mom, a.bn_per_entry, a.rows_t, a.rows_o, (q % a.bn_gx) * 256 + (int)threadIdx.x, q / a.bn_gx);
  } else assemble_bwd_lds_body(a.asmb_dc, (int)(b - b6));
}
__global__ __launch_bounds__(256) void vae_leaf_kernel(unsigned int b0, unsigned int b1, unsigned int b2, unsigned int b3, unsigned int b4,
                                                       unsigned int b5, unsigned int b6, LeafArgs a) {
  vae_leaf_dispatch(blockIdx.x, b0, b1, b2, b3, b4, b5, b6, a);
}

struct LeafRanges { unsigned int b0, b1, b2, b3, b4, b5, b6; };
template <bool G_X2>
__global__ __launch_bounds__(256) void vae_tail_kernel(const GemmTNArgs* __restrict__ probs, const TnMixedMeta* __restrict__ meta,
                                                       const unsigned int nwg, const LeafRanges r, const LeafArgs a) {
  extern __shared__ __attribute__((aligned(16))) char smem[];
  if (blockIdx.x >= nwg) { vae_leaf_dispatch(blockIdx.x - nwg, r.b0, r.b1, r.b2, r.b3, r.b4, r.b5, r.b6, a); return; }
  gemm_tn_mixed_item<G_X2>(probs, meta->item[blockIdx.x], smem);
}

int sln_vae_leaf_fits(const VaeLeaf& a) {
  if (g_sln_deterministic) return 0;
  const EncAssembleBwd& e = a.enc;
  if (e.O <= 0 || a.pred_rows <= 0) return 0;
  if (!(e.rows_obj > 0 && e.rows_angle > 0 && (e.n_attr == 0 || e.rows_attr > 0))) return 0;
  if ((long)e.rows_obj * e.n_obj + (long)e.rows_attr * e.n_attr + (long)e.rows_angle * e.n_angle > ASSEMBLE_LDS_MAX_FLOATS) return 0;
  if (a.pred_table_rows <= 0 || (long)a.pred_table_rows * a.n_pdc > EMBED_LDS_MAX_FLOATS || (long)a.pred_table_rows * a.n_pec > EMBED_LDS_MAX_FLOATS)
    return 0;
  if (a.n_attr_dc > 0 && (a.attr_table_rows <= 0 || (long)a.attr_table_rows * a.n_attr_dc > EMBED_LDS_MAX_FLOATS)) return 0;
  if (a.n_pdc <= 0 || a.n_pec <= 0 || e.n_box <= 0) return 0;
  if (a.dec.dx0) {
    const DecAssembleBwd& d = a.dec;
    if (d.dz || d.O != e.O || d.n_obj <= 0 || !(d.rows_obj > 0 && (d.n_attr == 0 || d.rows_attr > 0)) || a.dec_ld < d.n_obj + d.n_attr) return 0;
    if ((long)d.rows_obj * d.n_obj + (long)d.rows_attr * d.n_attr > ASSEMBLE_LDS_MAX_FLOATS) return 0;
  }
  return 1;
}

static unsigned int leaf_build(const VaeLeaf& v, LeafArgs& a, LeafRanges& rg, size_t& lds_out) {
  std::memset(&a, 0, sizeof(a));
  const EncAssembleBwd& e = v.enc;
  AssembleBwdLds& l = a.asmb;
  l.dx0 = e.dx0; l.ld = e.n_obj + e.n_attr + e.n_box + e.n_angle; l.O = e.O;
  int k = 0;
  l.seg[k++] = EmbSeg{e.objs, e.d_obj_emb, e.n_obj, e.rows_obj, 0, 0};
  if (e.n_attr > 0) l.seg[k++] = EmbSeg{e.attrs, e.d_attr_emb, e.n_attr, e.rows_attr, e.n_obj, 0};
  l.seg[k++] = EmbSeg{e.angles, e.d_angle_emb, e.n_angle, e.rows_angle, e.n_obj + e.n_attr + e.n_box, 0};
  l.nseg = k;
  int off = 0;
  for (int s = 0; s < l.nseg; ++s) { l.seg[s].lds0 = off; off += l.seg[s].rows * l.seg[s].n; }
  l.lds_floats = off;
  l.rows_per_block = l.O <= 8192 ? 16 : 64;
  a.box = e; a.box_gx = sln_cdiv(e.n_box, CB);
  const int rpb = embed_rows_per_block();
  a.pdc = LeafEmbedJob{v.pidx, v.d_pdc, v.d_pred_dc, v.ld_pdc, v.col0_pdc, v.pred_rows, v.n_pdc, v.pred_table_rows, rpb};
  a.pec = LeafEmbedJob{v.pidx, v.d_pec, v.d_pred_ec, v.ld_pec, v.col0_pec, v.pred_rows, v.n_pec, v.pred_table_rows, rpb};
  if (v.n_attr_dc > 0) a.attr = LeafEmbedJob{v.attr_idx, v.d_attr, v.d_attr_dc, v.ld_attr, v.col0_attr, e.O, v.n_attr_dc, v.attr_table_rows, rpb};
  a.bn_tab = v.bn_tab; a.bn_n = v.bn_n; a.bn_per_entry = v.bn_independent ? 1 : 0; a.bn_gx = sln_cdiv(v.bn_max_c > 0 ? v.bn_max_c : 1, 256);
  a.rows_t = v.pred_rows; a.rows_o = e.O; a.mom = v.bn_momentum;
  const unsigned int n_bn = v.bn_n > 0 ? (unsigned int)a.bn_gx * (unsigned int)(a.bn_per_entry ? v.bn_n : 1) : 0;
  const unsigned int n_asm = (unsigned int)sln_cdiv(l.O, l.rows_per_block);
  const unsigned int n_box = (unsigned int)a.box_gx * (unsigned int)sln_cdiv(e.O, BOX_ROWS);
  const unsigned int n_pred = (unsigned int)sln_cdiv(v.pred_rows, rpb);
  const unsigned int n_attr = v.n_attr_dc > 0 ? (unsigned int)sln_cdiv(e.O, rpb) : 0;
  const unsigned int b0 = n_asm, b1 = b0 + n_box, b2 = b1 + n_pred, b3 = b2 + n_pred, b4 = b3 + n_attr, b5 = b4 + n_bn;
  const unsigned int b6 = b5 + (v.bn_update ? n_bn : 0);
  unsigned int n_dasm = 0;
  if (v.dec.dx0) {
    AssembleBwdLds& d = a.asmb_dc;
    d.dx0 = v.dec.dx0; d.ld = v.dec_ld; d.O = v.dec.O;
    int kd = 0;
    d.seg[kd++] = EmbSeg{v.dec.objs, v.dec.d_obj_emb, v.dec.n_obj, v.dec.rows_obj, 0, 0};
    if (v.dec.n_attr > 0) d.seg[kd++] = EmbSeg{v.dec.attrs, v.dec.d_attr_emb, v.dec.n_attr, v.dec.rows_attr, v.dec.n_obj, 0};
    d.nseg = kd;
    int offd = 0;
    for (int s = 0; s < d.nseg; ++s) { d.seg[s].lds0 = offd; offd += d.seg[s].rows * d.seg[s].n; }
    d.lds_floats = offd;
    d.rows_per_block = d.O <= 8192 ? 16 : 64;
    n_dasm = (unsigned int)sln_cdiv(d.O, d.rows_per_block);
  }
  const unsigned int tot = b6 + n_dasm;
  size_t lds = sizeof(float) * 7 * RL * CB;
  auto grow = [&lds](long floats) { if (sizeof(float) * (size_t)floats > lds) lds = sizeof(float) * (size_t)floats; };
  grow(l.lds_floats); grow((long)v.pred_table_rows * v.n_pdc); grow((long)v.pred_table_rows * v.n_pec);
  if (v.n_attr_dc > 0) grow((long)v.attr_table_rows * v.n_attr_dc);
  grow(a.asmb_dc.lds_floats);
  rg = LeafRanges{b0, b1, b2, b3, b4, b5, b6};
  lds_out = lds;
  return tot;
}

int sln_launch_vae_leaf(const VaeLeaf& v, hipStream_t st) {
  if (!sln_vae_leaf_fits(v)) return -1;
  LeafArgs a; LeafRanges r; size_t lds = 0;
  const unsigned int tot = leaf_build(v, a, r, lds);
  hipLaunchKernelGGL(vae_leaf_kernel, dim3(tot), dim3(256), lds, st, r.b0, r.b1, r.b2, r.b3, r.b4, r.b5, r.b6, a);
  SLN_CHECK_LAUNCH();
  return 0;
}

int sln_vae_tail_init() {
  int r = (int)hipFuncSetAttribute(reinterpret_cast<const void*>(&vae_tail_kernel<true>), hipFuncAttributeMaxDynamicSharedMemorySize, 160 * 1024);
  if (!r) r = (int)hipFuncSetAttribute(reinterpret_cast<const void*>(&vae_tail_kernel<false>), hipFuncAttributeMaxDynamicSharedMemorySize, 160 * 1024);
  return r;
}

int sln_launch_vae_tail(const GemmTNArgs* dev_probs, const TnMixedMeta* dev_meta, int blocks, bool x2, double flops, const VaeLeaf& v,
                        hipStream_t st) {
  if (blocks < 0 || !sln_vae_leaf_fits(v)) return -1;
  LeafArgs a; LeafRanges r; size_t lds = 0;
  const unsigned int tot = leaf_build(v, a, r, lds);
  const size_t smem = tn_smem_bytes(64, 64);
  if (lds > smem) return -1;
  { const int e = sln_gemm_init(); if (e) return e; }
  SlnProfScope prof(SLN_FAM_GEMM_TN, flops, st);
  if (x2) hipLaunchKernelGGL((vae_tail_kernel<true>), dim3((unsigned int)blocks + tot), dim3(256), smem, st, dev_probs, dev_meta, (unsigned int)blocks, r, a);
  else hipLaunchKernelGGL((vae_tail_kernel<false>), dim3((unsigned int)blocks + tot), dim3(256), smem, st, dev_probs, dev_meta, (unsigned int)blocks, r, a);
  SLN_CHECK_LAUNCH();
  return 0;
}

int sln_launch_add2(const float* a, int lda, const float* b, int ldb, int rows, int cols, float* out, int ldo, hipStream_t st) {
  const long n = (long)rows * cols;
  if (n <= 0) return 0;
  hipLaunchKernelGGL(add2_kernel, dim3((unsigned)((n + 255) / 256)), dim3(256), 0, st, a, lda, b, ldb, rows, cols, out, ldo);
  SLN_CHECK_LAUNCH();
  return 0;
}

#include "vae_multi.h"
namespace {

template <int XT, int YT>
__global__ __launch_bounds__(XT* YT) void scatter_avg_fwd_multi_kernel(const MScatterFwd* __restrict__ tab) {
  const MScatterFwd& a = tab[blockIdx.z];
  if ((int)blockIdx.x >= a.gx || (int)blockIdx.y >= a.gy) return;
  scatter_avg_fwd_v4_body<XT, YT>(a.A2, a.ld, a.H, a.D, a.bn, a.g, a.O, a.g.T, a.pooled);
}
template <int XT, int YT, int RPT, int NIT>
__global__ __launch_bounds__(XT* YT) void scatter_avg_bwd_multi_kernel(const MScatterBwd* __restrict__ tab) {
  const MScatterBwd& a = tab[blockIdx.z];
  if ((int)blockIdx.x >= a.gx || (int)blockIdx.y >= a.gy) return;
  scatter_avg_bwd_v4_body<XT, YT, RPT, NIT>(a.dM, a.dP, a.lddp, a.dpcol0, a.A2, a.ld, a.H, a.D, a.bn, a.g, a.T, a.g2, a.gsums, a.cstride);
}
template <int XT, int YT>
__global__ __launch_bounds__(XT* YT) void gather_bwd_multi_kernel(const MGatherBwd* __restrict__ tab) {
  const MGatherBwd& a = tab[blockIdx.z];
  if ((int)blockIdx.x >= a.gx || (int)blockIdx.y >= a.gy) return;
  gather_bwd_v4_body<XT, YT>(a.dG, a.ldg, a.D, a.g, a.O, a.g.T, a.add1, a.ldadd1, a.xprev, a.ldx, a.bn, a.masked, a.out, a.ldo, a.gsums, a.cstride);
}
__global__ __launch_bounds__(CB* RL) void mask_gstats_multi_kernel(const MMaskGstats* __restrict__ tab) {
  const MMaskGstats& a = tab[blockIdx.z];
  if ((int)blockIdx.x >= a.gx || (int)blockIdx.y >= a.gy) return;
  mask_gstats_body(a.d1, a.ld1, a.d2, a.ld2, a.xprev, a.ldx, a.bn, a.rows, a.cols, a.out, a.ldo, a.gsums, a.cstride);
}
__global__ void dec_assemble_multi_kernel(const MDecAssemble* __restrict__ tab) {
  const MDecAssemble& a = tab[blockIdx.z];
  if ((int)blockIdx.x >= a.gx) return;
  dec_assemble_body(a.a);
}
__global__ void dec_assemble_bwd_multi_kernel(const MDecAssembleBwd* __restrict__ tab) {
  const MDecAssembleBwd& a = tab[blockIdx.z];
  if ((int)blockIdx.x >= a.gx) return;
  dec_assemble_bwd_body(a.a);
}
struct MAsmLds { AssembleBwdLds a; int gx, pad_; };
static_assert(sizeof(MAsmLds) <= SLN_ASM_BLOB && sizeof(MDecAssembleBwd) <= SLN_ASM_BLOB, "SLN_ASM_BLOB too small");
__global__ __launch_bounds__(256) void assemble_bwd_lds_multi_kernel(const char* __restrict__ tab) {
  const MAsmLds& a = *reinterpret_cast<const MAsmLds*>(tab + (size_t)blockIdx.z * SLN_ASM_BLOB);
  if ((int)blockIdx.x >= a.gx) return;
  assemble_bwd_lds_body(a.a, (int)blockIdx.x);
}
__global__ void dec_assemble_bwd_plain_multi_kernel(const char* __restrict__ tab) {
  const MDecAssembleBwd& a = *reinterpret_cast<const MDecAssembleBwd*>(tab + (size_t)blockIdx.z * SLN_ASM_BLOB);
  if ((int)blockIdx.x >= a.gx) return;
  dec_assemble_bwd_body(a.a);
}
__global__ void embed_gather_multi_kernel(const MEmbedGather* __restrict__ tab) {
  const MEmbedGather& a = tab[blockIdx.z];
  if ((int)blockIdx.x >= a.gx) return;
  embed_gather_body(a.idx, a.emb, a.rows, a.n, a.out, blockIdx.x);
}
template <typename IdxT, int V>
__global__ __launch_bounds__(V == MV_EMBED_DET ? 1024 : 256) void embed_bwd_multi_kernel(const MEmbedBwd* __restrict__ tab) {
  const MEmbedBwd& a = tab[blockIdx.z];
  if ((int)blockIdx.x >= a.gx || (int)blockIdx.y >= a.gy) return;
  const IdxT* idx = static_cast<const IdxT*>(a.idx);
  if (V == MV_EMBED_DET) embed_bwd_det_body<IdxT>(idx, a.d, a.ld, a.col0, a.rows, a.n, a.d_emb);
  else if (V == MV_EMBED_LDS) embed_bwd_lds_body<IdxT>(idx, a.d, a.ld, a.col0, a.rows, a.n, a.table_rows, a.rows_per_block, a.d_emb, (int)blockIdx.x);
  else embed_bwd_body<IdxT>(idx, a.d, a.ld, a.col0, a.rows, a.n, a.d_emb);
}
__global__ void add2_multi_kernel(const MAdd2* __restrict__ tab) {
  const MAdd2& a = tab[blockIdx.z];
  if ((int)blockIdx.x >= a.gx) return;
  add2_body(a.a, a.lda, a.b, a.ldb, a.rows, a.cols, a.out, a.ldo);
}
__global__ void copy2d_multi_kernel(const MAdd2* __restrict__ tab) {
  const MAdd2& a = tab[blockIdx.z];
// ... 203 lines not shown
```

### include/sln_hip.h

```cpp
#ifndef SLN_HIP_H
#define SLN_HIP_H

#include <stdint.h>

#ifdef __cplusplus
extern "C" {
#endif

#define SLN_E_BADARG (-1)
#define SLN_E_UNSUPPORTED (-2)
#define SLN_E_STATE (-3)
#define SLN_E_NOGPU (-4)
#define SLN_E_NOMEM (-5)
#define SLN_E_CAPTURE (-6)

int sln_version(void);
const char* sln_build_arch(void);
int sln_device_ok(void);


typedef struct SlnVaeConfig {
  int embedding_dim;
  int gconv_num_layers;
  int recurrent;
// ... 31 lines not shown
  float* flat_params; float* flat_grads; float* adam_m; float* adam_v; int64_t n_flat;
} SlnVaeTensors;

typedef struct SlnVaeBatch {
  const int64_t* objs;
  const int64_t* triples;
  const float*   boxes;
  const int64_t* angles;
  const int64_t* attributes;
  int O, T;
} SlnVaeBatch;

typedef struct SlnVae SlnVae;

int sln_vae_create(const SlnVaeConfig* cfg, SlnVae** out);
void sln_vae_destroy(SlnVae* h);
int64_t sln_vae_workspace_bytes(const SlnVae* h, int max_objs, int max_triples);
int sln_vae_bind(SlnVae* h, const SlnVaeTensors* t, void* workspace, int64_t workspace_bytes,
                 int max_objs, int max_triples);

int sln_vae_set_batch(SlnVae* h, const SlnVaeBatch* b, void* stream);
int sln_vae_check_batch(SlnVae* h, void* stream);

int sln_vae_encoder(SlnVae* h, float* mu, float* logvar, int training, void* stream);
int sln_vae_decoder(SlnVae* h, const float* z, float* boxes_pred, float* angles_pred, int training, void* stream);
int sln_vae_forward(SlnVae* h, const float* eps, float* mu, float* logvar, float* z_out, float* boxes_pred,
                    float* angles_pred, int training, void* stream);

int sln_vae_loss(SlnVae* h, const float* boxes_pred, const float* angles_pred, const float* mu,
                 const float* logvar, float kl_weight, float* losses_out, int with_grads, void* stream);

int sln_vae_decoder_backward(SlnVae* h, const float* d_boxes_pred, const float* d_angles_pred, float* dz, void* stream);
int sln_vae_encoder_backward(SlnVae* h, const float* d_mu, const float* d_logvar, void* stream);
int sln_vae_backward(SlnVae* h, void* stream);

int sln_vae_params_changed(SlnVae* h);
int sln_vae_zero_grad(SlnVae* h, void* stream);
int sln_vae_adam_step(SlnVae* h, float lr, void* stream);
int sln_vae_adam_reset(SlnVae* h, int64_t step, void* stream);
int sln_vae_adam_get_step(SlnVae* h, int64_t* step_out, void* stream);
int sln_vae_set_grad_guard(SlnVae* h, float* slot);
int sln_vae_seed(SlnVae* h, uint64_t seed, uint64_t offset, void* stream);
int sln_vae_last_eps(SlnVae* h, float* eps_out, void* stream);
int sln_vae_randn(SlnVae* h, float* out, int64_t n, void* stream);
int sln_layout_heatmap(const float* boxes_pred, int64_t n_trials, int O, int box_dim, int container_size, int clip_coor, float* counts,
                       void* stream);

enum { SLN_TRAIN_BACKWARD = 0, SLN_TRAIN_FULL = 1, SLN_TRAIN_UPTO_DECODER = 2, SLN_TRAIN_ENCODER_BWD = 3 };
int sln_vae_set_training(SlnVae* h, int training);
int sln_vae_set_gemm_precision(SlnVae* h, int mode);
int sln_vae_train_step(SlnVae* h, const float* eps, float kl_weight, float lr, float* losses_out, int use_graph,
                       int with_adam, void* stream);

typedef struct SlnVaeGroup SlnVaeGroup;
typedef struct SlnVaeGroupIO {
  int rows_total;
  const int* row0_host;
  const float* z;
  float* boxes_pred;
  float* angles_pred;
  float* d_boxes_pred;
  float* d_angles_pred;
  float* dz;
  const float* sgd_step;
} SlnVaeGroupIO;
int sln_vae_group_create(SlnVae* const* engines, int R, const SlnVaeGroupIO* io, SlnVaeGroup** out);
int sln_vae_group_decoder(SlnVaeGroup* g, void* stream);
int sln_vae_group_decoder_backward(SlnVaeGroup* g, void* stream);
int sln_vae_group_fused_params(const SlnVaeGroup* g, const float** params, int64_t* numel, int max);
int sln_vae_group_launches(const SlnVaeGroup* g, int* fwd, int* bwd, int* single_room_fallbacks);
int64_t sln_vae_group_transposes(const SlnVaeGroup* g);
void sln_vae_group_destroy(SlnVaeGroup* g);

int sln_debug_side_stream(void* stream, int* index, int* overlapped);
int sln_side_stream_prepare(void* stream);
int sln_side_stream_forget(void* stream);

int sln_prof_enable(int enable);
int sln_set_deterministic(int on);
int sln_get_deterministic(void);
int sln_set_store_policy(int bits);
int sln_get_store_policy(void);
int sln_parse_store_policy_env(const char* value, int dflt);
int sln_debug_tn_plan(const int* R, const int* Nout, const int* Kin, int n, int* rows_per_block, int* items, int max_items);
int sln_debug_tn_plan_mixed(const int* R, const int* Nout, const int* Kin, const int* gathers, int n, int* rows_per_block, int* items,
                            int max_items);
int sln_prof_read(double* ms_by_family, double* work_by_family, int64_t* launches_by_family, int n_families);

int64_t sln_vae_tap(SlnVae* h, int layer, int what, float* dst, void* stream);

int64_t sln_gconv_workspace_bytes(int D, int H, int Dout, int O, int T, int num_layers);
int sln_gconv_forward(int D, int H, int Dout, int num_layers, int n_modules, int batch_norm, const SlnVaeUnit* units_host,
                      const float* obj_vecs, const float* pred_vecs, const int64_t* edges, int O, int T, int training, void* workspace,
                      int64_t workspace_bytes, float* new_obj, float* new_pred, void* stream);

int sln_gconv_net_create(int D, int H, int Dout, int num_layers, int recurrent, int batch_norm, SlnVae** out);
int sln_gconv_net_set_edges(SlnVae* h, const int64_t* edges, int O, int T, void* stream);
int sln_gconv_net_forward(SlnVae* h, const float* obj_vecs, const float* pred_vecs, float* new_obj, float* new_pred, int training,
                          void* stream);
int sln_gconv_net_backward(SlnVae* h, const float* d_new_obj, const float* d_new_pred, float* d_obj_vecs, float* d_pred_vecs,
                           void* stream);

int sln_linear_forward(const float* x, int M, int K, const float* W, const float* bias, float* y, int N, double* sums,
                       int tile, void* stream);
int sln_linear_wgrad(const float* g, const float* x, int R, int N, int K, float* dW, float* db, void* stream);

typedef struct SlnDbgBn {
  const double* sums;
  const double* gsums;
  const float* gamma;
  const float* beta;
  const float* rmean;
  const float* rvar;
  int cstride;
  int mode;
  float n_rows;
  float eps;
} SlnDbgBn;
typedef struct SlnDbgSeg {
  const float* x1;
  const float* x2;
  int ld1, ld2, c1, c2, len, which, coef, pad_;
  SlnDbgBn bn;
} SlnDbgSeg;
typedef struct SlnDbgOperand {
  SlnDbgSeg seg[3];
  const int* idx_a;
  const int* idx_b;
  int nseg, pad_;
} SlnDbgOperand;
typedef struct SlnDbgGemmNT {
  SlnDbgOperand A;
  const float* W;
  const float* bias;
  float* Y;
  const float* addend;
  const float* xprev;
  double* osums;
  double* ogsums;
  SlnDbgBn obn;
  int M, N, K, ldw, ldy, ycol0, ldadd, addcol0, ocstride, ldx, xcol0, epi, tile, pad_;
} SlnDbgGemmNT;
typedef struct SlnDbgGemmTN {
  SlnDbgOperand G, X;
  float* dW;
  float* db;
  const float* sgd_step;
  int lddw, R, Nout, Kin, rows_per_block, pad_;
} SlnDbgGemmTN;
typedef struct SlnDbgNTRoute { int body, multi, amode, threads; } SlnDbgNTRoute;
int sln_debug_gemm_nt(const SlnDbgGemmNT* desc, int n, int* grouped, void* stream);
int sln_debug_gemm_tn(const SlnDbgGemmTN* desc, int n, int multi, void* stream);
int sln_debug_gemm_tn_mixed(const SlnDbgGemmTN* desc, int n, void* stream);
int sln_debug_gemm_nt_route(const SlnDbgGemmNT* desc, SlnDbgNTRoute* out);
int sln_debug_gemm_nt_half(const SlnDbgGemmNT* desc, int terms, void* stream);
int sln_debug_gemm_nt_half_takes(const SlnDbgGemmNT* desc);
int sln_debug_gemm_sizes(int* out, int max);

typedef struct SlnDbgCsr {
  int* s; int* p; int* o; int* deg; float* invdeg; int* rowptr; int* cursor; int* ent;
  int T, O;
} SlnDbgCsr;
int sln_debug_vae_csr(const int64_t* triples, int num_preds, int edges_only, int deg_is_zero, const SlnDbgCsr* g, int* err, void* stream);
typedef struct SlnDbgEdge {
  SlnDbgCsr g;
  SlnDbgBn bn;
// ... 329 lines not shown
```

Before: 36630 graphs/s (scene-graph VAE fwd+loss+bwd+Adam).

## Add bf16x3 split-precision MFMA path for TN weight-gradient GEMMs

Adds a TN (weight-gradient) GEMM body that splits each fp32 operand into three bf16 pieces, writes them to LDS and runs bf16 32x32x16 MFMAs with transposed LDS reads. This emulates near-fp32 accuracy on matrix cores in place of the fp32 path. The path is on by default, selected by an env/API switch, and is disabled in deterministic mode and for SGD-fused or keep_f32 problems. The grouped multi-room path marks its problems keep_f32, so it keeps the old kernel. It trades extra conversion work and six MFMAs per k-step for higher matrix throughput, with a small change in numerics.

```diff
diff --git a/3d_sln_amd/_lib.py b/3d_sln_amd/_lib.py
--- a/3d_sln_amd/_lib.py
+++ b/3d_sln_amd/_lib.py
@@ -221,6 +221,9 @@
     "sln_set_store_policy": (C.c_int, [C.c_int]),
     "sln_get_store_policy": (C.c_int, []),
     "sln_parse_store_policy_env": (C.c_int, [C.c_char_p, C.c_int]),
+    "sln_set_tn_split": (C.c_int, [C.c_int]),
+    "sln_get_tn_split": (C.c_int, []),
+    "sln_parse_tn_split_env": (C.c_int, [C.c_char_p, C.c_int]),
     "sln_debug_tn_plan": (C.c_int, [C.c_void_p, C.c_void_p, C.c_void_p, C.c_int, C.c_void_p, C.c_void_p, C.c_int]),
     "sln_debug_tn_plan_mixed": (C.c_int, [C.c_void_p, C.c_void_p, C.c_void_p, C.c_void_p, C.c_int, C.c_void_p, C.c_void_p, C.c_int]),
     "sln_prof_read": (C.c_int, [C.c_void_p, C.c_void_p, C.c_void_p, C.c_int]),
diff --git a/3d_sln_amd/csrc/gemm_bodies.h b/3d_sln_amd/csrc/gemm_bodies.h
--- a/3d_sln_amd/csrc/gemm_bodies.h
+++ b/3d_sln_amd/csrc/gemm_bodies.h
@@ -1343,9 +1343,255 @@
 }
 
 
-template <bool G_X2>
+typedef __bf16 sln_bf16x8 __attribute__((ext_vector_type(8)));
+typedef short sln_s16x4 __attribute__((ext_vector_type(4)));
+typedef __attribute__((address_space(3))) sln_s16x4* sln_lds_s16x4p;
+
+__device__ __forceinline__ unsigned tn_cvt_pk_bf16(float lo, float hi) {
+  unsigned r;
+  asm("v_cvt_pk_bf16_f32 %0, %1, %2" : "=v"(r) : "v"(lo), "v"(hi));
+  return r;
+}
+__device__ __forceinline__ void tn_split2(float a, float b, unsigned& p1, unsigned& p2, unsigned& p3) {
+  p1 = tn_cvt_pk_bf16(a, b);
+  a -= __uint_as_float(p1 << 16); b -= __uint_as_float(p1 & 0xffff0000u);
+  p2 = tn_cvt_pk_bf16(a, b);
+  a -= __uint_as_float(p2 << 16); b -= __uint_as_float(p2 & 0xffff0000u);
+  p3 = tn_cvt_pk_bf16(a, b);
+}
+__device__ __forceinline__ sln_bf16x8 tn_tr_frag(const char* p) {
+  const sln_s16x4 lo = __builtin_amdgcn_ds_read_tr16_b64_v4i16((sln_lds_s16x4p)(p));
+  const sln_s16x4 hi = __builtin_amdgcn_ds_read_tr16_b64_v4i16((sln_lds_s16x4p)(p + 4 * 128));
+  return __builtin_bit_cast(sln_bf16x8, __builtin_shufflevector(lo, hi, 0, 1, 2, 3, 4, 5, 6, 7));
+}
+
+template <bool G_X2, bool XG>
+__device__ __forceinline__ void gemm_tn_split_body(const GemmTNArgs& a, const int bx, const int by, char* smem) {
+  constexpr int BM = 64, BN = 64;
+  constexpr int TPR = 16, RPP = 16;
+  constexpr int ROWB = 128, IMG = BK * ROWB, OPB = 3 * IMG, BUFB = 2 * OPB;
+  static_assert(BK == 32 && 2 * BUFB == 2 * BK * (BM + TN_PAD + BN + TN_PAD) * 4, "the bf16 images fill the fp32 tiles' LDS (tn_smem_bytes)");
+  float4* coefG = reinterpret_cast<float4*>(smem);
+  float4* coefX = coefG + BM;
+  char* img = reinterpret_cast<char*>(coefX + BN);
+
+  const int tid = threadIdx.x, lane = tid & 63, wave = tid >> 6;
+  const int tiles_k = (a.Kin + BN - 1) / BN;
+  const int n0 = (bx / tiles_k) * BM, k0 = (bx % tiles_k) * BN;
+  const int rbeg = by * a.rows_per_block;
+  const int rend = min(a.R, rbeg + a.rows_per_block);
+
+  float* coefGp = reinterpret_cast<float*>(coefG);
+  if (tid < BM) {
+    const int c = tid;
+    const float4 v = coef_for_col(a.G, n0 + c);
+    if (G_X2) { coefGp[c] = v.x; coefGp[BM + c] = v.y; coefGp[2 * BM + c] = v.z; coefGp[3 * BM + c] = v.w; }
+    else coefG[c] = v;
+  } else if (tid < BM + BN) {
+    const int c = tid - BM;
+    coefX[c] = coef_for_col(a.X, k0 + c);
+  }
+
+  const int ca = 4 * (tid % TPR), ra0 = tid / TPR;
+  const ColSel gs = pick_col(a.G, n0 + ca);
+  const ColSel xs = pick_col(a.X, k0 + ca);
+
+  const int ntiles = (rend - rbeg + BK - 1) / BK;
+  const int last = ntiles - 1;
+  constexpr int NST = 2;
+  float4 g1[NST][2], g2[NST][2], x1[NST][2];
+  const float4 z4 = make_float4(0.f, 0.f, 0.f, 0.f);
+  const int* x_ip = xs.which == 2 ? a.X.idx_b : a.X.idx_a;
+  if (x_ip == nullptr) x_ip = a.X.idx_a ? a.X.idx_a : a.X.idx_b;
+  const float* g_x2 = gs.x2 ? gs.x2 : gs.x1;
+  const int g_ld2 = gs.x2 ? gs.ld2 : gs.ld1;
+  int xi[NST][2];
+  auto iload = [&](int rt, auto stage) {
+    constexpr int S = decltype(stage)::value;
+#pragma unroll
+    for (int p = 0; p < 2; ++p) xi[S][p] = ldi(x_ip + min(rbeg + rt * BK + ra0 + RPP * p, rend - 1));
+  };
+  auto gload = [&](int rt, int rt_idx, auto stage) {
+    constexpr int S = decltype(stage)::value;
+#pragma unroll
+    for (int p = 0; p < 2; ++p) {
+      const int row = min(rbeg + rt * BK + ra0 + RPP * p, rend - 1);
+      g1[S][p] = ld4(gs.x1 + (size_t)row * gs.ld1);
+      if (G_X2) g2[S][p] = ld4(g_x2 + (size_t)row * g_ld2);
+    }
+#pragma unroll
+    for (int p = 0; p < 2; ++p) {
+      const int row = min(rbeg + rt * BK + ra0 + RPP * p, rend - 1);
+      const int r = XG ? (xs.which ? xi[S][p] : row) : row;
+      x1[S][p] = ld4(xs.x1 + (size_t)r * xs.ld1);
+    }
+    if (XG) iload(rt_idx, stage);
+  };
+  float4 dbacc = z4;
+  float4 cG[4], cX[4];
+  const int woff = ra0 * ROWB + ((2 * ca) ^ (((ra0 >> 1) & 1) << 6));
+  auto put = [&](char* dst, float4 t) __attribute__((always_inline)) {
+    uint2 q1, q2, q3;
+    tn_split2(t.x, t.y, q1.x, q2.x, q3.x);
+    tn_split2(t.z, t.w, q1.y, q2.y, q3.y);
+    *reinterpret_cast<uint2*>(dst) = q1;
+    *reinterpret_cast<uint2*>(dst + IMG) = q2;
+    *reinterpret_cast<uint2*>(dst + 2 * IMG) = q3;
+  };
+  auto pieceG = [&](int rt, int buf, int p, auto stage) __attribute__((always_inline)) {
+    constexpr int S = decltype(stage)::value;
+    const int rl = ra0 + RPP * p;
+    const bool v = (rbeg + (rt + 1) * BK + rl) < rend;
+    float4 t = G_X2 ? xform_planar(g1[S][p], g2[S][p], *reinterpret_cast<const float4*>(coefGp + ca),
+                                   *reinterpret_cast<const float4*>(coefGp + BM + ca), *reinterpret_cast<const float4*>(coefGp + 2 * BM + ca),
+                                   *reinterpret_cast<const float4*>(coefGp + 3 * BM + ca))
+                    : xform1(g1[S][p], cG);
+    t.x = v ? t.x : 0.f; t.y = v ? t.y : 0.f; t.z = v ? t.z : 0.f; t.w = v ? t.w : 0.f;
+    dbacc.x += t.x; dbacc.y += t.y; dbacc.z += t.z; dbacc.w += t.w;
+    put(img + (buf ^ 1) * BUFB + p * RPP * ROWB + woff, t);
+    __builtin_amdgcn_sched_barrier(0);
+    const int row = min(rbeg + min(rt + 3, last) * BK + rl, rend - 1);
+    g1[S][p] = ld4(gs.x1 + (size_t)row * gs.ld1);
+    if (G_X2) g2[S][p] = ld4(g_x2 + (size_t)row * g_ld2);
+  };
+  auto pieceX = [&](int rt, int buf, int p, auto stage) __attribute__((always_inline)) {
+    constexpr int S = decltype(stage)::value;
+    put(img + (buf ^ 1) * BUFB + OPB + p * RPP * ROWB + woff, xform1(x1[S][p], cX));
+    __builtin_amdgcn_sched_barrier(0);
+    const int row = min(rbeg + min(rt + 3, last) * BK + ra0 + RPP * p, rend - 1);
+    const int r = XG ? (xs.which ? xi[S][p] : row) : row;
+    x1[S][p] = ld4(xs.x1 + (size_t)r * xs.ld1);
+  };
+  auto pieceI = [&](int rt, int p, auto stage) __attribute__((always_inline)) {
+    constexpr int S = decltype(stage)::value;
+    if (XG) xi[S][p] = ldi(x_ip + min(rbeg + min(rt + 5, last) * BK + ra0 + RPP * p, rend - 1));
+  };
+
+  f32x16 acc[2];
+#pragma unroll
+  for (int i = 0; i < 2; ++i)
+#pragma unroll
+    for (int r = 0; r < 16; ++r) acc[i][r] = 0.f;
+
+  using S0 = std::integral_constant<int, 0>; using S1 = std::integral_constant<int, 1>;
+  if (XG) { iload(0, S0{}); iload(min(1, last), S1{}); }
+  gload(0, min(2, last), S0{});
+  gload(min(1, last), min(3, last), S1{});
+  __syncthreads();
+#pragma unroll
+  for (int j = 0; j < 4; ++j) { if (!G_X2) cG[j] = coefG[ca + j]; cX[j] = coefX[ca + j]; }
+  pieceG(-1, 1, 0, S0{}); pieceG(-1, 1, 1, S0{}); pieceX(-1, 1, 0, S0{}); pieceX(-1, 1, 1, S0{});
+  if (XG) { pieceI(-1, 0, S0{}); pieceI(-1, 1, S0{}); }
+  __syncthreads();
+  const int lrow = lane & 31, lk = lane >> 5;
+  const int wr = wave >> 1, wc = wave & 1;
+  const int tq = (lane >> 2) & 3, tp = lane & 3;
+  const int rbase = (16 * wr + 8 * lk + tq) * ROWB + 32 * ((lane >> 4) & 1) + 8 * tp;
+  const int aG0 = rbase + 64 * (tq >> 1), aG1 = rbase + 64 * ((tq >> 1) ^ 1), aX = OPB + rbase + 64 * (wc ^ (tq >> 1));
+  sln_bf16x8 fg[3][2], fx[3];
+  using P1 = std::integral_constant<int, 0>; using P2 = std::integral_constant<int, 1>; using P3 = std::integral_constant<int, 2>;
+  auto rdG = [&](int buf, auto part) __attribute__((always_inline)) {
+    constexpr int P = decltype(part)::value;
+    fg[P][0] = tn_tr_frag(img + buf * BUFB + P * IMG + aG0);
+    fg[P][1] = tn_tr_frag(img + buf * BUFB + P * IMG + aG1);
+  };
+  auto rdX = [&](int buf, auto part) __attribute__((always_inline)) {
+    constexpr int P = decltype(part)::value;
+    fx[P] = tn_tr_frag(img + buf * BUFB + P * IMG + aX);
+  };
+  rdG(0, P1{}); rdX(0, P3{});
+#define SLN_SB __builtin_amdgcn_sched_barrier(0)
+  auto mma2 = [&](auto gp, auto xp, auto&& hook) __attribute__((always_inline)) {
+    constexpr int GP = decltype(gp)::value, XP = decltype(xp)::value;
+    acc[0] = __builtin_amdgcn_mfma_f32_32x32x16_bf16(fg[GP][0], fx[XP], acc[0], 0, 0, 0);
+    acc[1] = __builtin_amdgcn_mfma_f32_32x32x16_bf16(fg[GP][1], fx[XP], acc[1], 0, 0, 0);
+    SLN_SB; hook(); SLN_SB;
+  };
+  auto sbody = [&](int rt, auto stage_next) __attribute__((always_inline)) {
+    const int buf = rt & 1;
+    rdG(buf, P3{}); rdX(buf, P1{});
+    SLN_SB;
+    mma2(P1{}, P3{}, [&]() __attribute__((always_inline)) { pieceG(rt, buf, 0, stage_next); });
+    mma2(P3{}, P1{}, [&]() __attribute__((always_inline)) { rdG(buf, P2{}); rdX(buf, P2{}); SLN_SB; pieceG(rt, buf, 1, stage_next); });
+    mma2(P2{}, P2{}, [&]() __attribute__((always_inline)) { pieceX(rt, buf, 0, stage_next); });
+    mma2(P1{}, P2{}, [&]() __attribute__((always_inline)) { pieceX(rt, buf, 1, stage_next); });
+    mma2(P2{}, P1{}, [&]() __attribute__((always_inline)) { pieceI(rt, 0, stage_next); pieceI(rt, 1, stage_next); });
+    mma2(P1{}, P1{}, [&]() __attribute__((always_inline)) {});
+    __syncthreads();
+    rdG(buf ^ 1, P1{}); rdX(buf ^ 1, P3{});
+    SLN_SB;
+  };
+#undef SLN_SB
+  for (int rt = 0; rt < ntiles; rt += 2) { sbody(rt, S1{}); sbody(rt + 1, S0{}); }
+
+  __syncthreads();
+  float* red = reinterpret_cast<float*>(img);
+  {
+    float* dst = red + (wave * 16) * 64 + lane;
+    if (wr == 0) {
+#pragma unroll
+      for (int r = 0; r < 16; ++r) dst[r * 64] = tn_acc_read(acc[1][r]);
+    } else {
+#pragma unroll
+      for (int r = 0; r < 16; ++r) dst[r * 64] = tn_acc_read(acc[0][r]);
+    }
+  }
+  __syncthreads();
+  {
+    const float* src = red + ((wave ^ 2) * 16) * 64 + lane;
+    const float sc = a.sgd_step != nullptr ? -a.sgd_step[0] : 1.f;
+    const int k = k0 + 32 * wc + lrow;
+    float* dcol = a.dW + min(k, a.Kin - 1);
+    const bool kv = k < a.Kin;
+    if (wr == 0) {
+#pragma unroll
+      for (int r = 0; r < 16; ++r) {
+        const float v = (tn_acc_read(acc[0][r]) + src[r * 64]) * sc;
+        const int n = n0 + (r & 3) + 8 * (r >> 2) + 4 * lk;
+        if (kv && n < a.Nout) sln_gatomic_add(dcol + (size_t)n * a.lddw, v);
+      }
+    } else {
+#pragma unroll
+      for (int r = 0; r < 16; ++r) {
+        const float v = (src[r * 64] + tn_acc_read(acc[1][r])) * sc;
+        const int n = n0 + 32 + (r & 3) + 8 * (r >> 2) + 4 * lk;
+        if (kv && n < a.Nout) sln_gatomic_add(dcol + (size_t)n * a.lddw, v);
+      }
+    }
+  }
+
+  if (a.db != nullptr && (bx % tiles_k) == 0) {
+#pragma unroll
+    for (int off = TPR; off < 64; off <<= 1) {
+      dbacc.x += __shfl_xor(dbacc.x, off, 64); dbacc.y += __shfl_xor(dbacc.y, off, 64);
+      dbacc.z += __shfl_xor(dbacc.z, off, 64); dbacc.w += __shfl_xor(dbacc.w, off, 64);
+    }
+    __syncthreads();
+    float4* dbs = reinterpret_cast<float4*>(red);
+    if (lane < TPR) dbs[wave * TPR + lane] = dbacc;
+    __syncthreads();
+    if (tid < TPR) {
+      const float4 p0 = dbs[tid], p1 = dbs[TPR + tid], p2 = dbs[2 * TPR + tid], p3 = dbs[3 * TPR + tid];
+      const int n = n0 + 4 * tid;
+      const float sb = a.sgd_step != nullptr ? -a.sgd_step[0] : 1.f;
+      if (n + 0 < a.Nout) sln_gatomic_add(a.db + n + 0, (((p0.x + p1.x) + p2.x) + p3.x) * sb);
+      if (n + 1 < a.Nout) sln_gatomic_add(a.db + n + 1, (((p0.y + p1.y) + p2.y) + p3.y) * sb);
+      if (n + 2 < a.Nout) sln_gatomic_add(a.db + n + 2, (((p0.z + p1.z) + p2.z) + p3.z) * sb);
+      if (n + 3 < a.Nout) sln_gatomic_add(a.db + n + 3, (((p0.w + p1.w) + p2.w) + p3.w) * sb);
+    }
+  }
+}
+
+__host__ __device__ __forceinline__ bool tn_split_takes(const GemmTNArgs& a) { return a.sgd_step == nullptr && a.keep_f32 == 0; }
+
+template <bool G_X2, bool SPLIT = false>
 __device__ __forceinline__ void gemm_tn_mixed_item(const GemmTNArgs* __restrict__ probs, const TnMultiItem it, char* smem) {
   if (it.prob < 0) return;
+  if (SPLIT && tn_split_takes(probs[it.prob])) {
+    if (it.xg) gemm_tn_split_body<G_X2, true>(probs[it.prob], it.tile, it.chunk, smem);
+    else gemm_tn_split_body<G_X2, false>(probs[it.prob], it.tile, it.chunk, smem);
+    return;
+  }
   if (it.xg) gemm_tn_body<64, 64, 2, 2, G_X2, true>(probs[it.prob], it.tile, it.chunk, smem);
   else gemm_tn_body<64, 64, 2, 2, G_X2, false>(probs[it.prob], it.tile, it.chunk, smem);
 }
diff --git a/3d_sln_amd/csrc/gemm_f32.hip b/3d_sln_amd/csrc/gemm_f32.hip
--- a/3d_sln_amd/csrc/gemm_f32.hip
+++ b/3d_sln_amd/csrc/gemm_f32.hip
@@ -157,6 +157,24 @@
   gemm_tn_mixed_item<G_X2>(probs, meta->item[blockIdx.x], smem);
 }
 
+template <bool G_X2, bool XG>
+__global__ __launch_bounds__(256) void gemm_tn_split_kernel(const GemmTNArgs a) {
+  extern __shared__ __attribute__((aligned(16))) char smem[];
+  gemm_tn_split_body<G_X2, XG>(a, blockIdx.x, blockIdx.y, smem);
+}
+template <bool G_X2, bool XG>
+__global__ __launch_bounds__(256) void gemm_tn_multi_split_kernel(const GemmTNArgs* __restrict__ probs, const TnMultiMeta* __restrict__ meta) {
+  extern __shared__ __attribute__((aligned(16))) char smem[];
+  TnMultiItem it = meta->item[blockIdx.x];
+  it.xg = XG ? 1 : 0;
+  gemm_tn_mixed_item<G_X2, true>(probs, it, smem);
+}
+template <bool G_X2>
+__global__ __launch_bounds__(256) void gemm_tn_mixed_split_kernel(const GemmTNArgs* __restrict__ probs, const TnMixedMeta* __restrict__ meta) {
+  extern __shared__ __attribute__((aligned(16))) char smem[];
+  gemm_tn_mixed_item<G_X2, true>(probs, meta->item[blockIdx.x], smem);
+}
+
 template <int BM, int BN, int WM, int WN, bool G_X2>
 int launch_tn(const GemmTNArgs& a, hipStream_t st) {
   const size_t smem = tn_smem_bytes(BM, BN);
@@ -164,6 +182,12 @@
   const int gy = sln_cdiv(a.R, a.rows_per_block);
   if (gx <= 0 || gy <= 0) return 0;
   if (!tn_supported(a)) return -1;
+  if (sln_tn_split_launch() && tn_split_takes(a)) {
+    if (tn_gathers(a)) hipLaunchKernelGGL((gemm_tn_split_kernel<G_X2, true>), dim3(gx, gy), dim3(256), smem, st, a);
+    else hipLaunchKernelGGL((gemm_tn_split_kernel<G_X2, false>), dim3(gx, gy), dim3(256), smem, st, a);
+    SLN_CHECK_LAUNCH();
+    return 0;
+  }
   if (tn_gathers(a)) hipLaunchKernelGGL((gemm_tn_kernel<BM, BN, WM, WN, G_X2, true>), dim3(gx, gy), dim3(256), smem, st, a);
   else hipLaunchKernelGGL((gemm_tn_kernel<BM, BN, WM, WN, G_X2, false>), dim3(gx, gy), dim3(256), smem, st, a);
   SLN_CHECK_LAUNCH();
@@ -238,6 +262,15 @@
 #undef SLN_SET_TNM
   if (!r) r = (int)hipFuncSetAttribute(reinterpret_cast<const void*>(&gemm_tn_mixed_kernel<true>), hipFuncAttributeMaxDynamicSharedMemorySize, 160 * 1024);
   if (!r) r = (int)hipFuncSetAttribute(reinterpret_cast<const void*>(&gemm_tn_mixed_kernel<false>), hipFuncAttributeMaxDynamicSharedMemorySize, 160 * 1024);
+#define SLN_SET_TNS(X2, XG)                                                                                       \
+  if (!r) r = (int)hipFuncSetAttribute(reinterpret_cast<const void*>(&gemm_tn_split_kernel<X2, XG>),             \
+                                       hipFuncAttributeMaxDynamicSharedMemorySize, 160 * 1024);                  \
+  if (!r) r = (int)hipFuncSetAttribute(reinterpret_cast<const void*>(&gemm_tn_multi_split_kernel<X2, XG>),       \
+                                       hipFuncAttributeMaxDynamicSharedMemorySize, 160 * 1024);
+  SLN_SET_TNS(true, true) SLN_SET_TNS(true, false) SLN_SET_TNS(false, true) SLN_SET_TNS(false, false)
+#undef SLN_SET_TNS
+  if (!r) r = (int)hipFuncSetAttribute(reinterpret_cast<const void*>(&gemm_tn_mixed_split_kernel<true>), hipFuncAttributeMaxDynamicSharedMemorySize, 160 * 1024);
+  if (!r) r = (int)hipFuncSetAttribute(reinterpret_cast<const void*>(&gemm_tn_mixed_split_kernel<false>), hipFuncAttributeMaxDynamicSharedMemorySize, 160 * 1024);
   if (!r) r = sln_gemm_group_init();
   if (!r) r = sln_vae_tail_init();
   done = r == 0;
@@ -413,11 +446,19 @@
 }
 
 int sln_launch_gemm_tn_multi(const GemmTNArgs* dev_probs, const TnMultiMeta* dev_meta, int blocks, bool x2, bool xg, double flops,
-                             hipStream_t st) {
+                             hipStream_t st, bool all_keep_f32) {
   if (blocks <= 0) return 0;
   SlnProfScope prof(SLN_FAM_GEMM_TN, flops, st);
   const size_t smem = tn_smem_bytes(64, 64);
   if (smem > 48 * 1024) { int r = sln_gemm_init(); if (r) return r; }
+  if (sln_tn_split_launch() && !all_keep_f32) {
+    if (x2 && xg) hipLaunchKernelGGL((gemm_tn_multi_split_kernel<true, true>), dim3(blocks), dim3(256), smem, st, dev_probs, dev_meta);
+    else if (x2) hipLaunchKernelGGL((gemm_tn_multi_split_kernel<true, false>), dim3(blocks), dim3(256), smem, st, dev_probs, dev_meta);
+    else if (xg) hipLaunchKernelGGL((gemm_tn_multi_split_kernel<false, true>), dim3(blocks), dim3(256), smem, st, dev_probs, dev_meta);
+    else hipLaunchKernelGGL((gemm_tn_multi_split_kernel<false, false>), dim3(blocks), dim3(256), smem, st, dev_probs, dev_meta);
+    SLN_CHECK_LAUNCH();
+    return 0;
+  }
   if (x2 && xg) hipLaunchKernelGGL((gemm_tn_multi_kernel<true, true>), dim3(blocks), dim3(256), smem, st, dev_probs, dev_meta);
   else if (x2) hipLaunchKernelGGL((gemm_tn_multi_kernel<true, false>), dim3(blocks), dim3(256), smem, st, dev_probs, dev_meta);
   else if (xg) hipLaunchKernelGGL((gemm_tn_multi_kernel<false, true>), dim3(blocks), dim3(256), smem, st, dev_probs, dev_meta);
@@ -431,6 +472,12 @@
   SlnProfScope prof(SLN_FAM_GEMM_TN, flops, st);
   const size_t smem = tn_smem_bytes(64, 64);
   if (smem > 48 * 1024) { int r = sln_gemm_init(); if (r) return r; }
+  if (sln_tn_split_launch()) {
+    if (x2) hipLaunchKernelGGL((gemm_tn_mixed_split_kernel<true>), dim3(blocks), dim3(256), smem, st, dev_probs, dev_meta);
+    else hipLaunchKernelGGL((gemm_tn_mixed_split_kernel<false>), dim3(blocks), dim3(256), smem, st, dev_probs, dev_meta);
+    SLN_CHECK_LAUNCH();
+    return 0;
+  }
   if (x2) hipLaunchKernelGGL((gemm_tn_mixed_kernel<true>), dim3(blocks), dim3(256), smem, st, dev_probs, dev_meta);
   else hipLaunchKernelGGL((gemm_tn_mixed_kernel<false>), dim3(blocks), dim3(256), smem, st, dev_probs, dev_meta);
   SLN_CHECK_LAUNCH();
diff --git a/3d_sln_amd/csrc/prof.hip b/3d_sln_amd/csrc/prof.hip
--- a/3d_sln_amd/csrc/prof.hip
+++ b/3d_sln_amd/csrc/prof.hip
@@ -13,6 +13,11 @@
   return (int)x;
 }
 int g_sln_store_policy = sln_parse_store_policy(std::getenv("SLN_STORE_POLICY"), SLN_STORE_DEFAULT);
+int sln_parse_tn_split(const char* v, int dflt) {
+  if (!v || (v[0] != '0' && v[0] != '1') || v[1] != 0) return dflt;
+  return v[0] - '0';
+}
+int g_sln_tn_split = sln_parse_tn_split(std::getenv("SLN_TN_SPLIT"), SLN_TN_SPLIT_DEFAULT);
 int g_sln_deterministic = [] { const char* v = std::getenv("SLN_DETERMINISTIC"); return (v && v[0] == '1') ? 1 : 0; }();
 
 namespace {
@@ -45,6 +50,13 @@
 }
 extern "C" int sln_get_store_policy(void) { return g_sln_store_policy; }
 extern "C" int sln_parse_store_policy_env(const char* value, int dflt) { return sln_parse_store_policy(value, dflt); }
+extern "C" int sln_set_tn_split(int word) {
+  if (word != SLN_TN_SPLIT_OFF && word != SLN_TN_SPLIT_ON) return SLN_E_BADARG;
+  g_sln_tn_split = word;
+  return 0;
+}
+extern "C" int sln_get_tn_split(void) { return g_sln_tn_split; }
+extern "C" int sln_parse_tn_split_env(const char* value, int dflt) { return sln_parse_tn_split(value, dflt); }
 extern "C" int sln_prof_enable(int enable) {
   g_sln_prof_on = enable != 0;
   return 0;
diff --git a/3d_sln_amd/csrc/sln_common.h b/3d_sln_amd/csrc/sln_common.h
--- a/3d_sln_amd/csrc/sln_common.h
+++ b/3d_sln_amd/csrc/sln_common.h
@@ -230,6 +230,11 @@
   else *p = v;
 }
 
+enum { SLN_TN_SPLIT_OFF = 0, SLN_TN_SPLIT_ON = 1, SLN_TN_SPLIT_DEFAULT = SLN_TN_SPLIT_ON };
+extern int g_sln_tn_split;
+extern int g_sln_deterministic;
+static inline bool sln_tn_split_launch() { return g_sln_tn_split == SLN_TN_SPLIT_ON && !g_sln_deterministic; }
+
 static inline int sln_cdiv(int a, int b) { return (a + b - 1) / b; }
 
 template <typename T>
diff --git a/3d_sln_amd/csrc/sln_gemm.h b/3d_sln_amd/csrc/sln_gemm.h
--- a/3d_sln_amd/csrc/sln_gemm.h
+++ b/3d_sln_amd/csrc/sln_gemm.h
@@ -28,6 +28,7 @@
   int lddw;
   int R, Nout, Kin;
   int rows_per_block;
+  int keep_f32;
   const float* sgd_step;
 };
 
@@ -43,7 +44,7 @@
 struct TnMixedMeta { int nprob, nblocks; TnMultiItem item[SLN_TN_MIXED_ITEMS]; };
 int sln_tn_multi_plan(GemmTNArgs* probs, int n, TnMultiMeta* meta, int* blocks, bool* x2, bool* xg, double* flops);
 int sln_launch_gemm_tn_multi(const GemmTNArgs* dev_probs, const TnMultiMeta* dev_meta, int blocks, bool x2, bool xg, double flops,
-                             hipStream_t st);
+                             hipStream_t st, bool all_keep_f32 = false);
 int sln_tn_mixed_plan(GemmTNArgs* probs, int n, TnMixedMeta* meta, int* blocks, bool* x2, double* flops);
 int sln_launch_gemm_tn_mixed(const GemmTNArgs* dev_probs, const TnMixedMeta* dev_meta, int blocks, bool x2, double flops, hipStream_t st);
 int sln_gemm_init();
diff --git a/3d_sln_amd/csrc/vae_engine.hip b/3d_sln_amd/csrc/vae_engine.hip
--- a/3d_sln_amd/csrc/vae_engine.hip
+++ b/3d_sln_amd/csrc/vae_engine.hip
@@ -123,6 +123,7 @@
   bool capturing = false, tn_upload_pending = false;
   int det_seen = 0;
   int store_seen = 0;
+  int split_seen = 0;
   long graph_captures = 0;
   bool tn_per_layer = false;
   int tn_slot_next[3] = {0, 0, 0};
@@ -1410,6 +1411,7 @@
   }
   if (h->det_seen != g_sln_deterministic) { h->det_seen = g_sln_deterministic; h->drop_graphs(); }
   if (h->store_seen != g_sln_store_policy) { h->store_seen = g_sln_store_policy; h->drop_graphs(); }
+  if (h->split_seen != g_sln_tn_split) { h->split_seen = g_sln_tn_split; h->drop_graphs(); }
   if (use_graph && st != nullptr) {
     hipGraphExec_t& ge = h->graph_exec[mode];
     if (!ge || h->graph_O[mode] != h->O || h->graph_T[mode] != h->T) {
@@ -1704,6 +1706,7 @@
       if (kind == SK_TN) {
         for (int r = 0; r < R; ++r) {
           GemmTNArgs t = recs[r].steps[s].tn;
+          t.keep_f32 = 1;
           if (io.sgd_step != nullptr && t.lddw == t.Kin) {
             for (const Unit& u : eng[r]->units)
               if (u.p.d_weight == t.dW && (t.db == nullptr || u.p.d_bias == t.db)) {
@@ -1819,7 +1822,7 @@
           if (tr_pending) { r = (int)hipStreamWaitEvent(main_st, ev_tr, 0); tr_pending = false; }
           break;
         case L_NT: r = sln_launch_gemm_nt_small_multi(static_cast<const GemmNTArgs*>(l.tab), l.tiles, l.count, l.variant, l.gx, l.maxK, l.flops, st); break;
-        case L_TN_MULTI: r = sln_launch_gemm_tn_multi(l.tn_probs, l.tn_meta, l.blocks, l.x2, l.xg, l.flops, st); break;
+        case L_TN_MULTI: r = sln_launch_gemm_tn_multi(l.tn_probs, l.tn_meta, l.blocks, l.x2, l.xg, l.flops, st, true); break;
         case L_TN_SINGLE: r = sln_launch_gemm_tn(singles[l.single].tn, st); break;
         case L_SINGLE_STEP: r = run_single(singles[l.single], st); break;
         case SK_SCATTER_FWD: r = sln_launch_scatter_avg_fwd_multi(static_cast<const MScatterFwd*>(l.tab), l.count, l.variant, l.gx, l.gy, st); break;
diff --git a/3d_sln_amd/csrc/vae_kernels.hip b/3d_sln_amd/csrc/vae_kernels.hip
--- a/3d_sln_amd/csrc/vae_kernels.hip
+++ b/3d_sln_amd/csrc/vae_kernels.hip
@@ -1356,6 +1356,13 @@
   extern __shared__ __attribute__((aligned(16))) char smem[];
   if (blockIdx.x >= nwg) { vae_leaf_dispatch(blockIdx.x - nwg, r.b0, r.b1, r.b2, r.b3, r.b4, r.b5, r.b6, a); return; }
   gemm_tn_mixed_item<G_X2>(probs, meta->item[blockIdx.x], smem);
+}
+template <bool G_X2>
+__global__ __launch_bounds__(256) void vae_tail_split_kernel(const GemmTNArgs* __restrict__ probs, const TnMixedMeta* __restrict__ meta,
+                                                             const unsigned int nwg, const LeafRanges r, const LeafArgs a) {
+  extern __shared__ __attribute__((aligned(16))) char smem[];
+  if (blockIdx.x >= nwg) { vae_leaf_dispatch(blockIdx.x - nwg, r.b0, r.b1, r.b2, r.b3, r.b4, r.b5, r.b6, a); return; }
+  gemm_tn_mixed_item<G_X2, true>(probs, meta->item[blockIdx.x], smem);
 }
 
 int sln_vae_leaf_fits(const VaeLeaf& a) {
@@ -1441,6 +1448,8 @@
 int sln_vae_tail_init() {
   int r = (int)hipFuncSetAttribute(reinterpret_cast<const void*>(&vae_tail_kernel<true>), hipFuncAttributeMaxDynamicSharedMemorySize, 160 * 1024);
   if (!r) r = (int)hipFuncSetAttribute(reinterpret_cast<const void*>(&vae_tail_kernel<false>), hipFuncAttributeMaxDynamicSharedMemorySize, 160 * 1024);
+  if (!r) r = (int)hipFuncSetAttribute(reinterpret_cast<const void*>(&vae_tail_split_kernel<true>), hipFuncAttributeMaxDynamicSharedMemorySize, 160 * 1024);
+  if (!r) r = (int)hipFuncSetAttribute(reinterpret_cast<const void*>(&vae_tail_split_kernel<false>), hipFuncAttributeMaxDynamicSharedMemorySize, 160 * 1024);
   return r;
 }
 
@@ -1453,6 +1462,12 @@
   if (lds > smem) return -1;
   { const int e = sln_gemm_init(); if (e) return e; }
   SlnProfScope prof(SLN_FAM_GEMM_TN, flops, st);
+  if (sln_tn_split_launch()) {
+    if (x2) hipLaunchKernelGGL((vae_tail_split_kernel<true>), dim3((unsigned int)blocks + tot), dim3(256), smem, st, dev_probs, dev_meta, (unsigned int)blocks, r, a);
+    else hipLaunchKernelGGL((vae_tail_split_kernel<false>), dim3((unsigned int)blocks + tot), dim3(256), smem, st, dev_probs, dev_meta, (unsigned int)blocks, r, a);
+    SLN_CHECK_LAUNCH();
+    return 0;
+  }
   if (x2) hipLaunchKernelGGL((vae_tail_kernel<true>), dim3((unsigned int)blocks + tot), dim3(256), smem, st, dev_probs, dev_meta, (unsigned int)blocks, r, a);
   else hipLaunchKernelGGL((vae_tail_kernel<false>), dim3((unsigned int)blocks + tot), dim3(256), smem, st, dev_probs, dev_meta, (unsigned int)blocks, r, a);
   SLN_CHECK_LAUNCH();
diff --git a/include/sln_hip.h b/include/sln_hip.h
--- a/include/sln_hip.h
+++ b/include/sln_hip.h
@@ -137,6 +137,9 @@
 int sln_set_store_policy(int bits);
 int sln_get_store_policy(void);
 int sln_parse_store_policy_env(const char* value, int dflt);
+int sln_set_tn_split(int word);
+int sln_get_tn_split(void);
+int sln_parse_tn_split_env(const char* value, int dflt);
 int sln_debug_tn_plan(const int* R, const int* Nout, const int* Kin, int n, int* rows_per_block, int* items, int max_items);
 int sln_debug_tn_plan_mixed(const int* R, const int* Nout, const int* Kin, const int* gathers, int n, int* rows_per_block, int* items,
                             int max_items);
```

Measured after the change: 37530 graphs/s (scene-graph VAE fwd+loss+bwd+Adam), median of 6. 2.5% higher.
